# Scuttie/Few-Shot-Prompt-Learning-for-Vision-Language-Models-in-Imbalanced-Datasets

Hardware: AMD Instinct MI355X
Metric: CoCoOp ViT-B/16 16-shot train-step images/sec at 1/2/4/8 GPUs; eval images/sec (higher is better)
Workload: dtype fp32s

## Files before the change

### few-shot-prompt-learning-for-vision-language-models-in-imbalanced-datasets_amd/_native.py

```python
from __future__ import annotations

import ctypes
import hashlib
import os
import sys

_PKG = os.path.dirname(os.path.abspath(__file__))
LIB_PATH = os.environ.get("CLIPK_LIB") or os.path.join(_PKG, "libclipk.so")
_ROOT = os.path.dirname(_PKG)


def source_files():
    csrc = os.path.join(_PKG, "csrc")
    names = sorted(n for n in os.listdir(csrc) if n.endswith((".hip", ".h")) or n == "Makefile")
    rel = [("csrc/" + n, os.path.join(csrc, n)) for n in names]
    return rel + [("include/clipk.h", os.path.join(_ROOT, "include", "clipk.h"))]


def source_digest():
    h = hashlib.sha256()
    for rel, path in source_files():
        with open(path, "rb") as f:
            h.update(f"{hashlib.sha256(f.read()).hexdigest()}  {rel}\n".encode())
    return h.hexdigest()

F32, F16, BF16, F32S = 0, 1, 2, 3
PREFIX_CLS_GROUP0 = 1
PREFIX_SPLIT = 2
PREFIX_OUT_SPLIT = 4
ATTN_SPLIT = 1
ATTN_OUT_SPLIT = 2
F32S16 = 4
SPLIT_SCALE = 64.0
EPI_BIAS, EPI_BIAS_RES, EPI_BIAS_QGELU, EPI_DQGELU, EPI_NONE = 0, 1, 2, 3, 4
A_QGELU = 0x100
QGELU_DERIV = 0x200
OUT_SPLIT, A_SPLIT = 0x400, 0x800
ADAM_ADAM, ADAM_ADAMW, ADAM_AMSGRAD = 0, 1, 2
COLOR_BRIGHTNESS, COLOR_CONTRAST, COLOR_SATURATION, COLOR_HUE, COLOR_GRAYSCALE = 1, 2, 3, 4, 5
COLOR_MAX_OPS, COLOR_DESC = 5, 12
CONV_RES, CONV_RELU, CONV_OUT_F32 = 1, 2, 4
PROF_NONE, PROF_GEMM_FC, PROF_GEMM_ALL, PROF_ATTN, PROF_LN, PROF_GEMM_DGELU = 0, 1, 2, 3, 4, 5

_P = ctypes.c_void_p
_I = ctypes.c_int
_L = ctypes.c_long
_F = ctypes.c_float
_S = ctypes.c_size_t
_D = ctypes.c_double
_U = ctypes.c_uint

SIGNATURES = {
    "clipk_version": (ctypes.c_char_p, []),
    "clipk_source_digest": (ctypes.c_char_p, []),
    "clipk_strerror": (ctypes.c_char_p, [_I]),
    "clipk_device_arch_ok": (_I, []),
    "clipk_gemm": (_I, [_I, _I, _I, _I, _I, _I, _P, _I, _P, _I, _P, _P, _I, _P, _I, _P, _P, _I, _I, _P]),
    "clipk_gemm_auto_splits": (_I, [_I, _I, _I, _I]),
    "clipk_gemm_splitk_ws_bytes": (_S, [_I, _I, _I]),
    "clipk_gemm_splitk": (_I, [_I, _I, _I, _I, _I, _I, _P, _I, _P, _I, _P, _P, _I, _P, _I, _P, _I, _P, _S, _P]),
    "clipk_gemm_set_config": (_I, [_I]),
    "clipk_split_pack": (_I, [_I, _I, _P, _I, _P, _P]),
    "clipk_split_lo_zero": (_I, [_I, _I, _P, _P, _P]),
    "clipk_split_hi16": (_I, [_I, _I, _P, _P, _P]),
    "clipk_gemm_ln": (_I, [_I, _I, _I, _I, _I, _P, _I, _P, _I, _P, _P, _I, _P, _I, _P, _P, _P, _P, _P]),
    "clipk_ln_stats_merge": (_I, [_I, _I, _P, _P, _P, _P, _P]),
    "clipk_gemm_ln_merge_fused": (_I, [_I, _I, _I, _I]),
    "clipk_gemm_split_tile_rows": (_I, [_I, _I, _I, _I, _I]),
    "clipk_gemm_t256_cost": (_D, [_I, _I, _I]),
    "clipk_gemm_ln_stats_split": (_I, [_I, _I, _I, _I, _I, _P, _I, _P, _I, _P, _P, _I, _P, _I, _P, _P, _P, _P]),
    "clipk_gemm_ln_gamma": (_I, [_I, _I, _I, _I, _I, _P, _I, _P, _I, _P, _P, _I, _P, _P, _P, _P, _P]),
    "clipk_gemm_ln_merge": (_I, [_I, _I, _I, _I, _I, _P, _I, _P, _I, _P, _P, _I, _P, _P, _P, _P, _P, _P, _P]),
    "clipk_image_resample": (_I, [_I, _I, _I, _P, _P, _P, _P, _P, _P, _I, _P, _P]),
    "clipk_image_color": (_I, [_I, _I, _P, _P, _P, _P, _P, _I, _P, _P]),
    "clipk_gemm_stamps": (_I, [_P, _S]),
    "clipk_layernorm_fwd": (_I, [_I, _I, _I, _P, _I, _P, _P, _P, _P, _I, _P, _P, _P]),
    "clipk_layernorm_bwd": (_I, [_I, _I, _I, _P, _I, _P, _I, _P, _P, _P, _P, _P, _I, _P, _P, _I, _P, _I, _P]),
    "clipk_layernorm_fwd_x": (_I, [_I, _I, _I, _I, _P, _I, _P, _P, _P, _P, _I, _P, _P, _P]),
    "clipk_layernorm_bwd_x": (_I, [_I, _I, _I, _I, _P, _I, _P, _I, _P, _P, _P, _P, _P, _I, _P, _P, _I, _P, _I, _P]),
    "clipk_layernorm_bwd_x2": (_I, [_I, _I, _I, _I, _P, _I, _P, _I, _P, _P, _P, _P, _P, _I, _I, _P, _P, _I, _P, _I, _P]),
    "clipk_attention_fwd": (_I, [_I, _I, _I, _I, _I, _P, _I, _P, _I, _P, _P]),
    "clipk_attention_fwd_ex": (_I, [_I, _I, _I, _I, _I, _P, _I, _P, _I, _P, _I, _P]),
    "clipk_attention_bwd": (_I, [_I, _I, _I, _I, _I, _I, _P, _I, _P, _I, _P, _I, _P, _P, _I, _P]),
    "clipk_im2col": (_I, [_I, _I, _I, _I, _I, _P, _P, _P]),
    "clipk_vit_embed_ln": (_I, [_I, _I, _I, _P, _P, _P, _P, _P, _P, _P]),
    "clipk_prompt_assemble": (_I, [_I, _I, _I, _I, _P, _P, _P, _L, _L, _P, _P, _P, _P]),
    "clipk_ctx_grad": (_I, [_I, _I, _I, _I, _I, _I, _P, _P, _P, _P]),
    "clipk_prompt_assemble_rows": (_I, [_I, _I, _I, _I, _I, _P, _P, _P, _P, _L, _L, _P, _P, _P, _P]),
    "clipk_ctx_grad_rows": (_I, [_I, _I, _I, _I, _P, _P, _P, _P, _P]),
    "clipk_ctx_bias_grad_rows": (_I, [_I, _I, _I, _I, _P, _P, _P, _P, _P, _P]),
    "clipk_attention_prefix_fwd": (_I, [_I, _I, _I, _I, _I, _P, _P, _I, _P, _I, _P, _I, _P, _P]),
    "clipk_attention_prefix_ws_bytes": (_S, [_I, _I, _I]),
    "clipk_attention_prefix_bwd": (_I, [_I, _I, _I, _I, _I, _I, _P, _P, _I, _P, _I, _P, _I, _P, _I, _P, _P,
                                        _I, _P, _S, _P]),
    "clipk_attention_prefix_fwd_ex": (_I, [_I, _I, _I, _I, _I, _P, _P, _I, _P, _I, _P, _I, _P, _I, _P]),
    "clipk_attention_prefix_bwd_ex": (_I, [_I, _I, _I, _I, _I, _I, _P, _P, _I, _P, _I, _P, _I, _P, _I, _P, _P,
                                           _I, _P, _S, _I, _P]),
    "clipk_cosine_logits_fwd": (_I, [_I, _I, _I, _I, _F, _P, _P, _P, _P, _P, _P]),
    "clipk_cosine_logits_bwd": (_I, [_I, _I, _I, _I, _F, _P, _P, _P, _P, _P, _P, _P]),
    "clipk_ce_loss": (_I, [_I, _I, _P, _P, _P, _F, _I, _F, _P, _P, _P]),
    "clipk_ce_loss_reduce": (_I, [_I, _I, _P, _P, _P, _F, _I, _F, _I, _P, _P, _P, _P]),
    "clipk_ce_loss_mix": (_I, [_I, _I, _P, _P, _P, _F, _P, _F, _I, _F, _I, _P, _P, _P, _P]),
    "clipk_mixup_images": (_I, [_I, _L, _P, _P, _P, _P, _F, _F, _P, _P]),
    "clipk_ntxent_ws_bytes": (_S, [_I, _I]),
    "clipk_ntxent_loss": (_I, [_I, _I, _P, _P, _F, _F, _P, _P, _P, _P, _P]),
    "clipk_src_head_ws_bytes": (_S, [_I, _I, _I]),
    "clipk_src_head": (_I, [_I, _I, _I, _P, _P, _P, _P, _P, _P, _P, _F, _I, _F, _F, _F, _F, _F, _P, _P, _P, _P, _P,
                            _P]),
    "clipk_probe_head_ws_bytes": (_S, [_I, _I, _I]),
    "clipk_probe_head": (_I, [_I, _I, _I, _P, _P, _P, _P, _P, _F, _I, _I, _F, _F, _P, _P, _P, _P, _P, _P]),
    "clipk_meta_net_fwd": (_I, [_I, _I, _I, _I, _P, _P, _P, _P, _P, _P, _P, _P]),
    "clipk_meta_net_fwd_norm": (_I, [_I, _I, _I, _I, _P, _P, _P, _P, _P, _P, _P, _P, _P]),
    "clipk_status_take": (_I, [_P, _P, _P]),
    "clipk_meta_net_bwd": (_I, [_I, _I, _I, _I, _P, _P, _P, _P, _P, _P, _P, _P, _P, _P]),
    "clipk_sgd_step": (_I, [_L, _P, _P, _P, _F, _F, _F, _I, _P]),
    "clipk_sgd_step_multi": (_I, [_I, _P, _P, _P, _P, _P, _F, _F, _F, _P]),
    "clipk_sgd_step_multi_scaled": (_I, [_I, _P, _P, _P, _P, _P, _F, _F, _F, _F, _P]),
    "clipk_sgd_step_multi_if": (_I, [_I, _P, _P, _P, _P, _P, _F, _F, _F, _F, _P, _I, _P]),
    "clipk_adam_step_multi": (_I, [_I, _P, _P, _P, _P, _P, _P, _P, _P, _D, _D, _D, _D, _D, _I, _F, _P, _I, _P]),
    "clipk_cast": (_I, [_I, _L, _P, _P, _P]),
    "clipk_rows_copy": (_I, [_I, _I, _P, _P, _P, _P, _P]),
    "clipk_vit_embed_ln_vpt": (_I, [_I, _I, _I, _I, _P, _P, _P, _P, _P, _P, _P, _P]),
    "clipk_rows_inject": (_I, [_I, _I, _I, _I, _P, _P, _P, _I, _P]),
    "clipk_rows_collect": (_I, [_I, _I, _I, _I, _P, _I, _P, _I, _I, _P, _P, _I, _I, _P]),
    "clipk_encoder_set_deep_prompts": (_I, [_P, _I, _I, _I, _P, _P, _P]),
    "clipk_encoder_set_input_rows": (_I, [_P, _I]),
    "clipk_encoder_set_ln_fold": (_I, [_P, _P]),
    "clipk_encoder_set_split": (_I, [_P, _I]),
    "clipk_encoder_set_split_target": (_I, [_P, _I]),
    "clipk_encoder_set_status": (_I, [_P, _P]),
    "clipk_lora_merge": (_I, [_I, _I, _I, _I, _U, _F, _I, _I, _P, _P, _P, _P, _P, _P]),
    "clipk_lora_wgrad_ws_bytes": (_S, [_I, _I, _I]),
    "clipk_lora_wgrad": (_I, [_I, _I, _I, _I, _I, _I, _F, _P, _P, _P, _P, _P, _P, _P, _P, _P, _P, _P, _S, _P]),
    "clipk_encoder_set_lora": (_I, [_P, _I, _I, _U, _F, _P, _P, _P, _P]),
    "clipk_vit_prompted_saved_bytes": (_S, [_P, _I, _I]),
    "clipk_vit_prompted_ws_bytes": (_S, [_P, _I, _I]),
    "clipk_vit_forward_prompted": (_I, [_P, _I, _P, _I, _P, _P, _P, _S, _P, _S, _P]),
    "clipk_vit_backward_prompted": (_I, [_P, _I, _I, _P, _P, _P, _P, _S, _P, _P, _S, _P]),
    "clipk_encoder_create": (_I, [_I, _I, _I, _I, _I, _I, _P, _P, _P]),
    "clipk_encoder_destroy": (None, [_P]),
    "clipk_text_saved_bytes": (_S, [_P, _I, _I]),
    "clipk_text_ws_bytes": (_S, [_P, _I, _I]),
    "clipk_text_forward": (_I, [_P, _I, _I, _P, _P, _P, _P, _S, _P, _S, _P]),
    "clipk_text_bwd_ws_bytes": (_S, [_P, _I, _I]),
    "clipk_text_backward": (_I, [_P, _I, _I, _P, _P, _P, _S, _P, _P, _S, _P]),
    "clipk_text_packed_saved_bytes": (_S, [_P, _I, _I, _I]),
    "clipk_text_packed_ws_bytes": (_S, [_P, _I, _I, _I]),
    "clipk_text_packed_bwd_ws_bytes": (_S, [_P, _I, _I, _I, _I]),
    "clipk_text_forward_packed": (_I, [_P, _I, _I, _I, _I, _I, _P, _P, _P, _P, _P, _P, _S, _P, _S, _P]),
    "clipk_text_backward_packed": (_I, [_P, _I, _I, _I, _I, _I, _P, _P, _P, _P, _P, _S, _P, _P, _S, _P]),
    "clipk_vision_create": (_I, [_I, _I, _I, _I, _I, _I, _I, _P, _P, _P]),
    "clipk_vit_ws_bytes": (_S, [_P, _I]),
    "clipk_vit_forward": (_I, [_P, _I, _P, _P, _P, _S, _P]),
    "clipk_conv2d_nhwc": (_I, [_I, _I, _I, _I, _I, _I, _I, _I, _P, _P, _P, _P, _P, _P, _P]),
    "clipk_im2col_3x3s2": (_I, [_I, _I, _I, _P, _P, _P]),
    "clipk_avgpool2_nhwc": (_I, [_I, _I, _I, _I, _I, _P, _P, _P]),
    "clipk_attnpool_ws_bytes": (_S, [_I, _I, _I, _I]),
    "clipk_attnpool": (_I, [_I, _I, _I, _I, _I, _I, _P, _P, _P, _P, _P, _P, _P, _P, _P, _P, _S, _P]),
    "clipk_resnet_create": (_I, [_I, _P, _I, _I, _I, _P, _I, _P]),
    "clipk_resnet_destroy": (None, [_P]),
    "clipk_resnet_ws_bytes": (_S, [_P, _I]),
    "clipk_resnet_forward": (_I, [_P, _I, _P, _P, _P, _S, _P]),
    "clipk_prof_enable": (_I, [_I]),
    "clipk_prof_read": (_I, [_P, _P, _P]),
    "clipk_prof_sites_enable": (_I, [_I]),
    "clipk_prof_sites_read": (_I, [_I, _P, _P, _P, _P, _P, _P]),
}

PROF_NAME_LEN = 32


def prof_sites_read(max_sites: int = 64):
    lib = load()
    names = ctypes.create_string_buffer(max_sites * PROF_NAME_LEN)
    ms = (ctypes.c_double * max_sites)()
    cnt = (ctypes.c_long * max_sites)()
    fl = (ctypes.c_double * max_sites)()
    by = (ctypes.c_double * max_sites)()
    n = ctypes.c_int()
    check(lib.clipk_prof_sites_read(max_sites, names, ms, cnt, fl, by, ctypes.byref(n)), "clipk_prof_sites_read")
    out = {}
    for i in range(n.value):
        nm = names.raw[i * PROF_NAME_LEN:(i + 1) * PROF_NAME_LEN].split(b"\0", 1)[0].decode()
        if cnt[i]:
            out[nm] = (ms[i], cnt[i], fl[i], by[i])
    return out

_lib = None


class ClipkError(RuntimeError):
    pass


def load():
    global _lib
    if _lib is not None:
        return _lib
    if not os.path.isfile(LIB_PATH):
        raise ClipkError(f"{LIB_PATH} is missing: the HIP extension is not built "
                         f"(run `python __graft_entry__.py` or `make -C csrc`). No CPU fallback exists.")
    lib = ctypes.CDLL(LIB_PATH)
    for name, (res, args) in SIGNATURES.items():
        fn = getattr(lib, name)
        fn.restype = res
        fn.argtypes = args
    built = lib.clipk_source_digest().decode()
    tree = source_digest()
    if built != tree:
        raise ClipkError(f"{LIB_PATH} was built from other sources than this tree (library digest {built[:16]}, "
                         f"tree {tree[:16]}): rebuild it (`python __graft_entry__.py` or `make -C csrc`)")
    _lib = lib
    return lib


def library_digest():
    return load().clipk_source_digest().decode()


def strerror(rc: int) -> str:
    return load().clipk_strerror(rc).decode()


def check(rc: int, what: str):
    if rc != 0:
        raise ClipkError(f"{what} failed: {strerror(rc)} (status {rc})")


def call(name: str, *args):
    rc = getattr(load(), name)(*args)
    check(rc, name)
    return rc


if __name__ == "__main__" and sys.argv[1:] == ["--digest-header"]:
    print(f'#define CLIPK_SOURCE_DIGEST "{source_digest()}"')
```

### few-shot-prompt-learning-for-vision-language-models-in-imbalanced-datasets_amd/csrc/attention_prefix.hip

```cpp
#include <cstdlib>

#include "attn_common.h"

namespace clipk {

constexpr int kValuChunkMin = 4;

static int chunk_env(const char* name, int def) {
  const char* e = getenv(name);
  const int v = e ? atoi(e) : def;
  return v >= 1 && v <= 16 ? v : def;
}
static int lds_slots();
static int fwd_chunk() { static int c = chunk_env("CLIPK_PREFIX_FWD_CHUNK", lds_slots() ? 4 : 8); return c; }
static int bwd_chunk() { static int c = chunk_env("CLIPK_PREFIX_BWD_CHUNK", 16); return c; }
static int prefix_num_cus() {
  static int n = 0;
  if (!n) {
    int dev = 0, v = 0;
    n = (hipGetDevice(&dev) == hipSuccess &&
         hipDeviceGetAttribute(&v, hipDeviceAttributeMultiprocessorCount, dev) == hipSuccess && v > 0)
            ? v
            : 256;
  }
// ... 698 lines not shown
__device__ __forceinline__ void f32_stage_prefix(const float* __restrict__ qkv, size_t row0, int P, int ldq, int col,
                                                 int W, float* sKp, float* sVp) {
  for (int i = threadIdx.x; i < P * 16; i += WPB * 64) {
    const int j = i >> 4, c = i & 15;
    const float* b = qkv + (row0 + j) * ldq + col + 4 * c;
    reinterpret_cast<f32x4*>(sKp)[i] = *reinterpret_cast<const f32x4*>(b + W);
    reinterpret_cast<f32x4*>(sVp)[i] = *reinterpret_cast<const f32x4*>(b + 2 * W);
  }
}
static size_t f32_prefix_lds(int P) { return (size_t)2 * P * 64 * sizeof(float); }

template <int WPB>
__global__ __launch_bounds__(WPB * 64) void attn_prefix_fwd_f32(
    int G, int P, int R, int ntiles, const int* __restrict__ tiles, const int* __restrict__ row_first, int H,
    int nchunk, int uc, const float* __restrict__ qkv, int ldq, float* __restrict__ out, int ldo,
    float* __restrict__ lse, int cls0) {
  extern __shared__ CLIPK_LDS_ALIGN float sPre[];
  float* const sKp = sPre;
  float* const sVp = sPre + P * 64;
  __shared__ CLIPK_LDS_ALIGN float sK[WPB][16 * 64], sV[WPB][16 * 64];
  int g, h, k, w;
  f32_block<WPB>(H, nchunk, g, h, k, w);
  const int W = H * 64;
  f32_stage_prefix<WPB>(qkv, (size_t)g * R, P, ldq, h * 64, W, sKp, sVp);
  __syncthreads();
  if (k >= nchunk) return;
  const int lane = threadIdx.x & 63, r = lane >> 2, s = lane & 3;
  float* sk = sK[w];
  float* sv = sV[w];
  const int u_end = min((k + 1) * uc, ntiles + 1);
  float qn[16], kn[16], vn[16];
  int t0n, nn, pren, rrn, firstn;
  auto fetch = [&](int u) {
    f32_unit(tiles, row_first, P, u, r, t0n, nn, pren, rrn, firstn);
    const float* qp = qkv + ((cls0 && u > 0 ? 0 : (size_t)g * R) + t0n + rrn) * ldq + h * 64 + kSl * s;
    ld16x(qp, qn);
    ld16x(qp + W, kn);
    ld16x(qp + 2 * W, vn);
  };
  if (k * uc < u_end) fetch(k * uc);
  for (int u = k * uc; u < u_end; ++u) {
    const int t0 = t0n, n = nn, pre = pren, rr = rrn, first = firstn;
    const size_t row = (size_t)g * R + t0 + rr;
    float q[16];
#pragma unroll
    for (int d = 0; d < 16; ++d) q[d] = qn[d] * kScale;
    st16x(sk + r * 64 + kSl * s, kn);
    st16x(sv + r * 64 + kSl * s, vn);
    lds_sync();
    if (u + 1 < u_end) fetch(u + 1);
    float sp[16], so[16], m = -INFINITY;
#pragma unroll
    for (int j = 0; j < 16; ++j) {
      if (j < pre) {
        float kv[16];
        ld16x(sKp + j * 64 + kSl * s, kv);
        sp[j] = quad_sum(dot16(q, kv));
        m = fmaxf(m, sp[j]);
      }
    }
#pragma unroll
    for (int j = 0; j < 16; ++j) {
      if (j < n) {
        float kv[16];
        ld16x(sk + j * 64 + kSl * s, kv);
        const float sc = quad_sum(dot16(q, kv));
        so[j] = (j <= rr && j >= first) ? sc : -INFINITY;
        m = fmaxf(m, so[j]);
      }
    }
    float l = 0.f, o[16];
#pragma unroll
    for (int d = 0; d < 16; ++d) o[d] = 0.f;
#pragma unroll
    for (int j = 0; j < 16; ++j) {
      if (j < pre) {
        float vv[16];
        ld16x(sVp + j * 64 + kSl * s, vv);
        const float p = __expf(sp[j] - m);
        l += p;
#pragma unroll
        for (int d = 0; d < 16; ++d) o[d] = fmaf(p, vv[d], o[d]);
      }
    }
#pragma unroll
    for (int j = 0; j < 16; ++j) {
      if (j < n) {
        float vv[16];
        ld16x(sv + j * 64 + kSl * s, vv);
        const float p = __expf(so[j] - m);
        l += p;
#pragma unroll
        for (int d = 0; d < 16; ++d) o[d] = fmaf(p, vv[d], o[d]);
      }
    }
    if (r < n) {
      const float inv = 1.0f / l;
#pragma unroll
      for (int d = 0; d < 16; ++d) o[d] *= inv;
      st16x(out + row * ldo + h * 64 + kSl * s, o);
      if (lse && s == 0) lse[row * H + h] = m + __logf(l);
    }
    lds_sync();
  }
}

template <int WPB, bool OS = false>
__global__ __launch_bounds__(WPB * 64, 2) void attn_prefix_bwd_f32(
    int G, int P, int R, int ntiles, const int* __restrict__ tiles, const int* __restrict__ row_first, int H,
    int nchunk, int uc, const float* __restrict__ qkv, int ldq, const float* __restrict__ o_fwd, int ldof,
    const float* __restrict__ dout, int lddo, const float* __restrict__ lse, float* __restrict__ dqkv, int lddq,
    float* __restrict__ part, int cls0) {
  extern __shared__ CLIPK_LDS_ALIGN float sPre[];
  float* const sKp = sPre;
  float* const sVp = sPre + P * 64;
  constexpr int RS = 68, PS = 33;
  __shared__ CLIPK_LDS_ALIGN float sA[WPB][16 * RS], sB[WPB][16 * RS];
  __shared__ CLIPK_LDS_ALIGN float sP[WPB][16 * PS], sS[WPB][16 * PS];
  int g, h, k, w;
  f32_block<WPB>(H, nchunk, g, h, k, w);
  const int W = H * 64;
  f32_stage_prefix<WPB>(qkv, (size_t)g * R, P, ldq, h * 64, W, sKp, sVp);
  __syncthreads();
  if (k >= nchunk) return;
  const int lane = threadIdx.x & 63, r = lane >> 2, s = lane & 3;
  float* sa = sA[w];
  float* sb = sB[w];
  float* sp = sP[w];
  float* ss = sS[w];
  float akp[16], avp[16];
#pragma unroll
  for (int d = 0; d < 16; ++d) { akp[d] = 0.f; avp[d] = 0.f; }
  const int u_end = min((k + 1) * uc, ntiles + 1);
  float qn[16], dOn[16], on[16], kn[16], vn[16], lin = 0.f;
  int t0n, nn, pren, rrn, firstn;
  auto fetch = [&](int u) {
    f32_unit(tiles, row_first, P, u, r, t0n, nn, pren, rrn, firstn);
    const size_t rw = (size_t)g * R + t0n + rrn;
    const float* qp = qkv + ((cls0 && u > 0 ? 0 : (size_t)g * R) + t0n + rrn) * ldq + h * 64 + kSl * s;
    ld16x(qp, qn);
    ld16x(dout + rw * lddo + h * 64 + kSl * s, dOn);
    ld16x(o_fwd + rw * ldof + h * 64 + kSl * s, on);
    ld16x(qp + W, kn);
    ld16x(qp + 2 * W, vn);
    lin = lse[rw * H + h];
  };
  if (k * uc < u_end) fetch(k * uc);
  for (int u = k * uc; u < u_end; ++u) {
    const int t0 = t0n, n = nn, pre = pren, rr = rrn, first = firstn;
    const bool qok = r < n;
    const size_t row = (size_t)g * R + t0 + rr;
    float q[16], dO[16];
#pragma unroll
    for (int d = 0; d < 16; ++d) {
      q[d] = qn[d] * kScale;
      dO[d] = dOn[d];
    }
    const float Di = quad_sum(dot16(dO, on));
    const float li = lin;
    st16x(sa + r * RS + kSl * s, kn);
    st16x(sb + r * RS + kSl * s, vn);
    lds_sync();
    if (u + 1 < u_end) fetch(u + 1);
    float dq[16];
#pragma unroll
    for (int d = 0; d < 16; ++d) dq[d] = 0.f;
    auto key = [&](const float* kr, const float* vr, bool ok, int col) {
      float kv[16], vv[16];
      ld16x(kr + kSl * s, kv);
      ld16x(vr + kSl * s, vv);
      const float sc = quad_sum(dot16(q, kv));
      const float dp = quad_sum(dot16(dO, vv));
      const float p = ok ? __expf(sc - li) : 0.f;
      const float ds = p * (dp - Di);
#pragma unroll
      for (int d = 0; d < 16; ++d) dq[d] = fmaf(ds, kv[d], dq[d]);
      if (s == 0) {
        sp[r * PS + col] = p;
        ss[r * PS + col] = ds;
      }
    };
    for (int j = 0; j < pre; ++j) key(sKp + j * 64, sVp + j * 64, qok, j);
    for (int j = 0; j < n; ++j) key(sa + j * RS, sb + j * RS, qok && j <= rr && j >= first, 16 + j);
    if (qok) {
#pragma unroll
      for (int d = 0; d < 16; ++d) dq[d] *= kScale;
      if constexpr (OS) st16x_split(dqkv + row * lddq + h * 64 + kSl * s, dq, s);
      else st16x(dqkv + row * lddq + h * 64 + kSl * s, dq);
    }
    st16x(sa + r * RS + kSl * s, q);
    st16x(sb + r * RS + kSl * s, dO);
    lds_sync();
    auto keysum = [&](int col, float* dk, float* dv) {
      for (int i = 0; i < n; ++i) {
        const float pv = sp[i * PS + col], dsv = ss[i * PS + col];
        float a[16], b[16];
        ld16x(sa + i * RS + kSl * s, a);
        ld16x(sb + i * RS + kSl * s, b);
#pragma unroll
        for (int d = 0; d < 16; ++d) {
          dk[d] = fmaf(dsv, a[d], dk[d]);
          dv[d] = fmaf(pv, b[d], dv[d]);
        }
      }
    };
    if (u == 0) {
      keysum(16 + r, akp, avp);
    } else {
      float dk[16], dv[16];
#pragma unroll
      for (int d = 0; d < 16; ++d) { dk[d] = 0.f; dv[d] = 0.f; }
      for (int i = 0; i < n; ++i) {
        const float pv = sp[i * PS + 16 + r], dsv = ss[i * PS + 16 + r];
        const float pp = sp[i * PS + r], dsp = ss[i * PS + r];
        float a[16], b[16];
        ld16x(sa + i * RS + kSl * s, a);
        ld16x(sb + i * RS + kSl * s, b);
#pragma unroll
        for (int d = 0; d < 16; ++d) {
          dk[d] = fmaf(dsv, a[d], dk[d]);
          dv[d] = fmaf(pv, b[d], dv[d]);
          akp[d] = fmaf(dsp, a[d], akp[d]);
          avp[d] = fmaf(pp, b[d], avp[d]);
        }
      }
      if (qok) {
        if constexpr (OS) {
          st16x_split(dqkv + row * lddq + W + h * 64 + kSl * s, dk, s);
          st16x_split(dqkv + row * lddq + 2 * W + h * 64 + kSl * s, dv, s);
        } else {
          st16x(dqkv + row * lddq + W + h * 64 + kSl * s, dk);
          st16x(dqkv + row * lddq + 2 * W + h * 64 + kSl * s, dv);
        }
      }
    }
    lds_sync();
  }
  if (r < P) {
    float* pb = part + (((size_t)g * nchunk + k) * 16 + r) * (2 * W) + h * 64 + kSl * s;
    st16x(pb, akp);
    st16x(pb + W, avp);
  }
}


struct Parts8 { s16x8 hi[2], lo[2]; };

__device__ __forceinline__ void ld_frag32(const float* p, f32x4 (&x)[4]) {
#pragma unroll
  for (int i = 0; i < 4; ++i) x[i] = *reinterpret_cast<const f32x4*>(p + 16 * i);
}
__device__ __forceinline__ void split_frag(const f32x4 (&x)[4], Parts8& o) {
#pragma unroll
  for (int kk = 0; kk < 2; ++kk) {
    f16x8 h, l;
#pragma unroll
    for (int j = 0; j < 2; ++j)
#pragma unroll
      for (int e = 0; e < 4; ++e) {
        const float v = x[2 * kk + j][e];
        const f16 hh = (f16)v;
        h[4 * j + e] = hh;
        l[4 * j + e] = (f16)(v - (float)hh);
      }
    o.hi[kk] = __builtin_bit_cast(s16x8, h);
    o.lo[kk] = __builtin_bit_cast(s16x8, l);
  }
}
__device__ __forceinline__ void st_parts(const Parts8& f, short* thi, short* tlo, int r16, int g4) {
#pragma unroll
  for (int i = 0; i < 4; ++i) {
    const int o = r16 * TRS + 16 * i + 4 * g4;
    const s16x8 h = f.hi[i >> 1], l = f.lo[i >> 1];
    const int b = 4 * (i & 1);
    *reinterpret_cast<s16x4*>(thi + o) = (s16x4){h[b], h[b + 1], h[b + 2], h[b + 3]};
    *reinterpret_cast<s16x4*>(tlo + o) = (s16x4){l[b], l[b + 1], l[b + 2], l[b + 3]};
  }
}
__device__ __forceinline__ f32x4 mfma32_s3(const Parts8& a, const Parts8& b, f32x4 c) {
#pragma unroll
  for (int kk = 0; kk < 2; ++kk) {
    c = mfma32_t<f16>(a.lo[kk], b.hi[kk], c);
    c = mfma32_t<f16>(a.hi[kk], b.lo[kk], c);
  }
#pragma unroll
  for (int kk = 0; kk < 2; ++kk) c = mfma32_t<f16>(a.hi[kk], b.hi[kk], c);
  return c;
}
__device__ __forceinline__ f32x4 mfma16_s3(s16x4 ah, s16x4 al, s16x4 bh, s16x4 bl, f32x4 c) {
  c = mfma16_t<f16>(al, bh, c);
  c = mfma16_t<f16>(ah, bl, c);
  return mfma16_t<f16>(ah, bh, c);
}
__device__ __forceinline__ void ld_prefix_parts(const float* p, bool ok, Parts8& o) {
  f32x4 x[4];
  ld_frag32(p, x);
#pragma unroll
  for (int i = 0; i < 4; ++i)
    if (!ok) x[i] = (f32x4){0.f, 0.f, 0.f, 0.f};
  split_frag(x, o);
}
constexpr int kSplitFwdWpc = 12, kSplitBwdWpc = 8;

template <int WPB, bool OS>
__global__ __launch_bounds__(WPB * 64) void attn_prefix_fwd_split(
    int G, int P, int R, int ntiles, const int* __restrict__ tiles, const int* __restrict__ row_first, int H,
    int nchunk, int uc, const float* __restrict__ qkv, int ldq, float* __restrict__ out, int ldo,
    float* __restrict__ lse, int cls0) {
  __shared__ CLIPK_LDS_ALIGN short sm[WPB][4][16 * TRS];
  const int lane = threadIdx.x & 63, w = threadIdx.x >> 6;
  const int r16 = lane & 15, g4 = lane >> 4;
  const int wid = blockIdx.x * WPB + w;
  if (wid >= G * nchunk * H) return;
  const int h = wid % H, k = (wid / H) % nchunk, g = wid / (H * nchunk);
  const int W = H * 64;
  short* sVpH = sm[w][0];
  short* sVpL = sm[w][1];
  short* sVoH = sm[w][2];
  short* sVoL = sm[w][3];
  const size_t gR = (size_t)g * R;
  const float* qh = qkv + h * 64 + 4 * g4;
  const int u_begin = k * uc, u_end = min((k + 1) * uc, ntiles + 1);
  const int tab = load_tile_table(tiles, ntiles, u_begin, lane);

  f32x4 qn[4], kn[4], vn[4];
  int firstn = 0;
  auto fetch = [&](int u) {
    int t0, n, pre;
    tile_info(tab, P, u, u_begin, t0, n, pre);
    const int rl = t0 + min(r16, n - 1);
    const float* qp = qh + ((cls0 && u > 0 ? 0 : gR) + rl) * ldq;
    ld_frag32(qp, qn);
    ld_frag32(qp + W, kn);
    ld_frag32(qp + 2 * W, vn);
    firstn = u == 0 ? 0 : row_first[rl] - t0;
  };
  if (u_begin < u_end) fetch(u_begin);
  Parts8 kp;
  {
    const bool pok = r16 < P;
    const float* pp = qh + (gR + (pok ? r16 : 0)) * ldq;
    Parts8 vp;
    ld_prefix_parts(pp + W, pok, kp);
    ld_prefix_parts(pp + 2 * W, pok, vp);
    st_parts(vp, sVpH, sVpL, r16, g4);
  }
  for (int u = u_begin; u < u_end; ++u) {
    int t0, n, pre;
    tile_info(tab, P, u, u_begin, t0, n, pre);
    const int first = firstn;
    const bool qok = r16 < n;
    Parts8 q, ko;
    {
      Parts8 vo;
      split_frag(qn, q);
      split_frag(kn, ko);
      split_frag(vn, vo);
      lds_fence();
      st_parts(vo, sVoH, sVoL, r16, g4);
    }
    const f32x4 z = {0.f, 0.f, 0.f, 0.f};
    const f32x4 sp = mfma32_s3(kp, q, z);
    const f32x4 so = mfma32_s3(ko, q, z);
    __builtin_amdgcn_sched_barrier(0);
    if (u + 1 < u_end) fetch(u + 1);
    float vp[4], vq[4], mx = -INFINITY;
#pragma unroll
    for (int r = 0; r < 4; ++r) {
      const int key = 4 * g4 + r;
      vp[r] = key < pre ? sp[r] * kScale : -INFINITY;
      vq[r] = (key <= r16 && key >= first) ? so[r] * kScale : -INFINITY;
      mx = fmaxf(mx, fmaxf(vp[r], vq[r]));
    }
    mx = xmax4(mx);
    float ep[4], eo[4], ps = 0.f;
#pragma unroll
    for (int r = 0; r < 4; ++r) {
      ep[r] = __expf(vp[r] - mx);
      eo[r] = __expf(vq[r] - mx);
      ps += ep[r] + eo[r];
    }
    ps = xsum4(ps);
    s16x4 bpH, bpL, boH, boL;
    split_pack4(ep[0] * kPScale, ep[1] * kPScale, ep[2] * kPScale, ep[3] * kPScale, bpH, bpL);
    split_pack4(eo[0] * kPScale, eo[1] * kPScale, eo[2] * kPScale, eo[3] * kPScale, boH, boL);
    const float inv = kPInv / ps;
    lds_fence();
    float* orow = out + (gR + t0 + r16) * ldo + h * 64;
#pragma unroll
    for (int t = 0; t < 4; ++t) {
      f32x4 o = mfma16_s3(tr_read(sVpH, 4 * g4, 16 * t, lane), tr_read(sVpL, 4 * g4, 16 * t, lane), bpH, bpL, z);
      o = mfma16_s3(tr_read(sVoH, 4 * g4, 16 * t, lane), tr_read(sVoL, 4 * g4, 16 * t, lane), boH, boL, o);
      store_acc16<OS>(orow, o * inv, t, qok, g4);
    }
    if (lse && g4 == 0 && qok) lse[(gR + t0 + r16) * H + h] = mx + __logf(ps);
  }
}

template <int WPB, bool OS>
__global__ __launch_bounds__(WPB * 64, 2) void attn_prefix_bwd_split(
    int G, int P, int R, int ntiles, const int* __restrict__ tiles, const int* __restrict__ row_first, int H,
    int nchunk, int uc, const float* __restrict__ qkv, int ldq, const float* __restrict__ dout, int lddo,
    const float* __restrict__ lse, float* __restrict__ dqkv, int lddq, float* __restrict__ part, int cls0) {
  __shared__ CLIPK_LDS_ALIGN short sm[WPB][8][16 * TRS];
  const int lane = threadIdx.x & 63, w = threadIdx.x >> 6;
  const int r16 = lane & 15, g4 = lane >> 4;
  const int wid = blockIdx.x * WPB + w;
  if (wid >= G * nchunk * H) return;
  const int h = wid % H, k = (wid / H) % nchunk, g = wid / (H * nchunk);
  const int W = H * 64;
  short* tKpH = sm[w][0];
  short* tKpL = sm[w][1];
  short* tKoH = sm[w][2];
  short* tKoL = sm[w][3];
  short* tQH = sm[w][4];
  short* tQL = sm[w][5];
  short* tDH = sm[w][6];
  short* tDL = sm[w][7];
  const size_t gR = (size_t)g * R;
  const float* qh = qkv + h * 64 + 4 * g4;
  const float* dh = dout + h * 64 + 4 * g4;
  const float* lse_h = lse + h;
  const int u_begin = k * uc, u_end = min((k + 1) * uc, ntiles + 1);
  const int tab = load_tile_table(tiles, ntiles, u_begin, lane);

  f32x4 qn[4], kn[4], vn[4], dn[4];
  float l2n = 0.f;
  int first2n = 0;
  auto fetch = [&](int u) {
    int t0, n, pre;
    tile_info(tab, P, u, u_begin, t0, n, pre);
    const int rl = t0 + min(r16, n - 1);
    const float* qp = qh + ((cls0 && u > 0 ? 0 : gR) + rl) * ldq;
    ld_frag32(qp, qn);
    ld_frag32(qp + W, kn);
    ld_frag32(qp + 2 * W, vn);
    ld_frag32(dh + (gR + rl) * lddo, dn);
    l2n = lse_h[(gR + rl) * H];
    first2n = u == 0 ? 0 : row_first[rl] - t0;
  };
  if (u_begin < u_end) fetch(u_begin);
  Parts8 kp, vp;
  {
    const bool pok = r16 < P;
    const float* pp = qh + (gR + (pok ? r16 : 0)) * ldq;
    ld_prefix_parts(pp + W, pok, kp);
    ld_prefix_parts(pp + 2 * W, pok, vp);
    st_parts(kp, tKpH, tKpL, r16, g4);
  }
  const f32x4 z = {0.f, 0.f, 0.f, 0.f};
  f32x4 dkp[4], dvp[4];
#pragma unroll
  for (int t = 0; t < 4; ++t) {
    dkp[t] = z;
    dvp[t] = z;
  }
  for (int u = u_begin; u < u_end; ++u) {
    int t0, n, pre;
    tile_info(tab, P, u, u_begin, t0, n, pre);
    const bool own_is_prefix = u == 0;
    const bool qok = r16 < n;
    const float l2 = l2n;
    const int first2 = first2n;
    f32x4 s1p, s2p, p1p, p2p, s1o, s2o, p1o, p2o;
    {
      Parts8 q, ko, vo, d;
      split_frag(qn, q);
      split_frag(kn, ko);
      split_frag(vn, vo);
      split_frag(dn, d);
      lds_fence();
      st_parts(q, tQH, tQL, r16, g4);
      st_parts(ko, tKoH, tKoL, r16, g4);
      st_parts(d, tDH, tDL, r16, g4);
      s1p = mfma32_s3(q, kp, z);
      s2p = mfma32_s3(kp, q, z);
      p1p = mfma32_s3(d, vp, z);
      p2p = mfma32_s3(vp, d, z);
      s1o = mfma32_s3(q, ko, z);
      s2o = mfma32_s3(ko, q, z);
      p1o = mfma32_s3(d, vo, z);
      p2o = mfma32_s3(vo, d, z);
    }
    __builtin_amdgcn_sched_barrier(0);
    if (u + 1 < u_end) fetch(u + 1);
    float P2p[4], P2o[4], Dsum = 0.f;
#pragma unroll
    for (int r = 0; r < 4; ++r) {
      const int j = 4 * g4 + r;
      P2p[r] = (qok && j < pre) ? __expf(s2p[r] * kScale - l2) : 0.f;
      P2o[r] = (qok && j <= r16 && j >= first2) ? __expf(s2o[r] * kScale - l2) : 0.f;
      Dsum += P2p[r] * p2p[r] + P2o[r] * p2o[r];
    }
    Dsum = xsum4(Dsum);
    s16x4 bTpH, bTpL, bToH, bToL;
    split_pack4(P2p[0] * (p2p[0] - Dsum), P2p[1] * (p2p[1] - Dsum), P2p[2] * (p2p[2] - Dsum),
                P2p[3] * (p2p[3] - Dsum), bTpH, bTpL);
    split_pack4(P2o[0] * (p2o[0] - Dsum), P2o[1] * (p2o[1] - Dsum), P2o[2] * (p2o[2] - Dsum),
                P2o[3] * (p2o[3] - Dsum), bToH, bToL);
    float P1p[4], P1o[4], dS1p[4], dS1o[4];
#pragma unroll
    for (int r = 0; r < 4; ++r) {
      const int i = 4 * g4 + r;
      const bool iok = i < n;
      const float Di = __shfl(Dsum, i, 64), l1 = __shfl(l2, i, 64);
      const int first1 = __shfl(first2, i, 64);
      P1p[r] = (iok && r16 < pre) ? __expf(s1p[r] * kScale - l1) : 0.f;
      P1o[r] = (iok && r16 <= i && r16 >= first1) ? __expf(s1o[r] * kScale - l1) : 0.f;
      dS1p[r] = P1p[r] * (p1p[r] - Di);
      dS1o[r] = P1o[r] * (p1o[r] - Di);
    }
    s16x4 bPpH, bPpL, bPoH, bPoL, bSpH, bSpL, bSoH, bSoL;
    split_pack4(P1p[0] * kPScale, P1p[1] * kPScale, P1p[2] * kPScale, P1p[3] * kPScale, bPpH, bPpL);
    split_pack4(P1o[0] * kPScale, P1o[1] * kPScale, P1o[2] * kPScale, P1o[3] * kPScale, bPoH, bPoL);
    split_pack4(dS1p[0], dS1p[1], dS1p[2], dS1p[3], bSpH, bSpL);
    split_pack4(dS1o[0], dS1o[1], dS1o[2], dS1o[3], bSoH, bSoL);
    lds_fence();
    float* orow = dqkv + (gR + t0 + r16) * lddq + h * 64;
    f32x4 acc[4];
#pragma unroll
    for (int t = 0; t < 4; ++t) {
      acc[t] = mfma16_s3(tr_read(tKpH, 4 * g4, 16 * t, lane), tr_read(tKpL, 4 * g4, 16 * t, lane), bTpH, bTpL, z);
      acc[t] = mfma16_s3(tr_read(tKoH, 4 * g4, 16 * t, lane), tr_read(tKoL, 4 * g4, 16 * t, lane), bToH, bToL, acc[t]);
    }
    store_acc64<OS>(orow, acc, kScale, qok, g4);
#pragma unroll
    for (int t = 0; t < 4; ++t) {
      const s16x4 aH = tr_read(tQH, 4 * g4, 16 * t, lane), aL = tr_read(tQL, 4 * g4, 16 * t, lane);
      dkp[t] = mfma16_s3(aH, aL, bSpH, bSpL, dkp[t]);
      acc[t] = mfma16_s3(aH, aL, bSoH, bSoL, z);
      if (own_is_prefix) dkp[t] += acc[t];
    }
    if (!own_is_prefix) store_acc64<OS>(orow + W, acc, kScale, qok, g4);
#pragma unroll
    for (int t = 0; t < 4; ++t) {
      const s16x4 aH = tr_read(tDH, 4 * g4, 16 * t, lane), aL = tr_read(tDL, 4 * g4, 16 * t, lane);
      dvp[t] = mfma16_s3(aH, aL, bPpH, bPpL, dvp[t]);
      acc[t] = mfma16_s3(aH, aL, bPoH, bPoL, z);
      if (own_is_prefix) dvp[t] += acc[t];
    }
    if (!own_is_prefix) store_acc64<OS>(orow + 2 * W, acc, kPInv, qok, g4);
  }
  float* pb = part + ((size_t)g * nchunk + k) * 16 * (2 * W);
  if (r16 < P) {
#pragma unroll
    for (int t = 0; t < 4; ++t) {
      float* dst = pb + (size_t)r16 * 2 * W + h * 64 + 16 * t + 4 * g4;
      *reinterpret_cast<f32x4*>(dst) = dkp[t] * kScale;
      *reinterpret_cast<f32x4*>(dst + W) = dvp[t] * kPInv;
    }
  }
}

template <typename TG>
__global__ __launch_bounds__(256) void prefix_kv_reduce(int P, int R, int W, int nchunk,
                                                        const float* __restrict__ part,
                                                        TG* __restrict__ dqkv, int lddq) {
  const int g = blockIdx.x / P, p = blockIdx.x % P;
  const int col = blockIdx.y * 256 + threadIdx.x;
  if (col >= 2 * W) return;
  const float* src = part + ((size_t)g * nchunk * 16 + p) * 2 * W + col;
  const size_t cs = (size_t)16 * 2 * W;
  float a0 = 0.f, a1 = 0.f, a2 = 0.f, a3 = 0.f;
  int k = 0;
  for (; k + 16 <= nchunk; k += 16) {
    float v[16];
#pragma unroll
    for (int i = 0; i < 16; ++i) v[i] = src[(k + i) * cs];
#pragma unroll
    for (int i = 0; i < 16; i += 4) {
      a0 += v[i];
      a1 += v[i + 1];
      a2 += v[i + 2];
      a3 += v[i + 3];
    }
  }
  for (; k + 4 <= nchunk; k += 4) {
    a0 += src[k * cs];
    a1 += src[(k + 1) * cs];
    a2 += src[(k + 2) * cs];
    a3 += src[(k + 3) * cs];
  }
  for (; k < nchunk; ++k) a0 += src[k * cs];
  const float acc = (a0 + a1) + (a2 + a3);
  dqkv[((size_t)g * R + p) * lddq + W + col] = (TG)acc;
}

__global__ __launch_bounds__(256) void prefix_kv_reduce_split(int P, int R, int W, int nchunk,
                                                              const float* __restrict__ part,
                                                              float* __restrict__ dqkv, int lddq) {
  const int g = blockIdx.x / P, p = blockIdx.x % P;
  const int col = blockIdx.y * 256 + threadIdx.x;
  if (col >= 2 * W) return;
  const float* src = part + ((size_t)g * nchunk * 16 + p) * 2 * W + col;
  const size_t cs = (size_t)16 * 2 * W;
  float a0 = 0.f, a1 = 0.f, a2 = 0.f, a3 = 0.f;
  int k = 0;
  for (; k + 16 <= nchunk; k += 16) {
    float v[16];
#pragma unroll
    for (int i = 0; i < 16; ++i) v[i] = src[(k + i) * cs];
#pragma unroll
    for (int i = 0; i < 16; i += 4) {
      a0 += v[i];
      a1 += v[i + 1];
      a2 += v[i + 2];
      a3 += v[i + 3];
    }
  }
  for (; k + 4 <= nchunk; k += 4) {
    a0 += src[k * cs];
    a1 += src[(k + 1) * cs];
    a2 += src[(k + 2) * cs];
    a3 += src[(k + 3) * cs];
  }
  for (; k < nchunk; ++k) a0 += src[k * cs];
  _Float16 hi, lo;
  split_parts((a0 + a1) + (a2 + a3), hi, lo);
  const int c = W + col;
  _Float16* grp = reinterpret_cast<_Float16*>(dqkv + ((size_t)g * R + p) * lddq + (c & ~7));
  grp[c & 7] = hi;
  grp[8 + (c & 7)] = lo;
}

template <typename T>
static int prefix_fwd(int G, int P, int R, int ntiles, const int* tiles, const int* row_first, int H,
                      const void* qkv, int ldq, void* out, int ldo, float* lse, hipStream_t st, int cls0) {
  if constexpr (sizeof(T) == 2) {
    const int uc = fwd_chunk();
    const int nchunk = n_chunks(ntiles, uc);
    const long waves = (long)G * nchunk * H;
    if (const int ns = lds_slots()) {
      const int wpb = lds_wpb();
      auto go = [&](auto kern) {
        hipLaunchKernelGGL(kern, dim3((waves + wpb - 1) / wpb), dim3(64 * wpb), 0, st, G, P, R, ntiles, tiles,
                           row_first, H, nchunk, uc, (const T*)qkv, ldq, (T*)out, ldo, lse, cls0);
      };
#define CLIPK_LDS_GO(K, T_, ...)                                                               \
  if (ns == 2) { if (wpb == 1) go(K<T_, 2, 1 __VA_ARGS__>); else if (wpb == 2) go(K<T_, 2, 2 __VA_ARGS__>); \
                 else go(K<T_, 2, 4 __VA_ARGS__>); }                                                 \
  else { if (wpb == 1) go(K<T_, 3, 1 __VA_ARGS__>); else if (wpb == 2) go(K<T_, 3, 2 __VA_ARGS__>);     \
         else go(K<T_, 3, 4 __VA_ARGS__>); }
      CLIPK_LDS_GO(attn_prefix_fwd_lds, T)
      CLIPK_CHECK_LAUNCH();
      return CLIPK_OK;
    }
    const int b = fwd_batch();
    const int wpb = prefix_wpb();
    auto go = [&](auto kern) {
      hipLaunchKernelGGL(kern, dim3((waves + wpb - 1) / wpb), dim3(64 * wpb), 0, st, G, P, R, ntiles, tiles,
                         row_first, H, nchunk, uc, (const T*)qkv, ldq, (T*)out, ldo, lse, cls0);
    };
    if (wpb == 8) {
      if (b == 1) go(attn_prefix_fwd_mfma<T, 1, 8>);
      else if (b == 2) go(attn_prefix_fwd_mfma<T, 2, 8>);
      else go(attn_prefix_fwd_mfma<T, 4, 8>);
    } else {
      if (b == 1) go(attn_prefix_fwd_mfma<T, 1>);
      else if (b == 2) go(attn_prefix_fwd_mfma<T, 2>);
      else go(attn_prefix_fwd_mfma<T, 4>);
    }
  } else {
    const int uc = f32_uc(G, ntiles, H, kF32FwdWpc);
    const int nchunk = n_chunks(ntiles, uc);
    auto go = [&](auto kern, int wpb) {
      const long blocks = (long)G * ((nchunk + wpb - 1) / wpb) * H;
      hipLaunchKernelGGL(kern, dim3(blocks), dim3(64 * wpb), f32_prefix_lds(P), st, G, P, R, ntiles, tiles, row_first,
                         H, nchunk, uc, (const float*)qkv, ldq, (float*)out, ldo, lse, cls0);
    };
    const int wpb = f32_wpb();
    if (wpb == 2) go(attn_prefix_fwd_f32<2>, 2);
    else if (wpb == 8) go(attn_prefix_fwd_f32<8>, 8);
    else go(attn_prefix_fwd_f32<4>, 4);
  }
  CLIPK_CHECK_LAUNCH();
  return CLIPK_OK;
}

template <typename T, typename TG, bool OS = false>
static int prefix_bwd(int G, int P, int R, int ntiles, const int* tiles, const int* row_first, int H,
                      const void* qkv, int ldq, const void* ofwd, int ldof, const void* dout, int lddo,
                      const float* lse, void* dqkv, int lddq, float* part, hipStream_t st, int cls0) {
  static_assert(!OS || (sizeof(T) == 4 && sizeof(TG) == 4), "pre-split dQ|dK|dV: the fp32 backward");
  constexpr bool mfma = sizeof(TG) == 2 && sizeof(T) == 2;
  const int uc = mfma ? bwd_uc(G, ntiles, H) : f32_uc(G, ntiles, H, kF32BwdWpc);
  const int nchunk = n_chunks(ntiles, uc);
  const long waves = (long)G * nchunk * H;
  if constexpr (mfma && __is_same(T, TG)) {
    if (const int ns = lds_slots()) {
      const int wpb = lds_wpb();
      auto go = [&](auto kern) {
        hipLaunchKernelGGL(kern, dim3((waves + wpb - 1) / wpb), dim3(64 * wpb), 0, st, G, P, R, ntiles, tiles,
                           row_first, H, nchunk, uc, (const T*)qkv, ldq, (const T*)dout, lddo, lse, (T*)dqkv,
                           lddq, part, cls0);
      };
      CLIPK_LDS_GO(attn_prefix_bwd_lds, T)
      CLIPK_CHECK_LAUNCH();
      const int W = H * 64;
      hipLaunchKernelGGL((prefix_kv_reduce<TG>), dim3(G * P, (2 * W + 255) / 256), dim3(256), 0, st, P, R, W,
                         nchunk, part, (TG*)dqkv, lddq);
      CLIPK_CHECK_LAUNCH();
      return CLIPK_OK;
    }
  }
  if constexpr (mfma) {
    const int wpb = prefix_wpb();
    auto go = [&](auto kern) {
      hipLaunchKernelGGL(kern, dim3((waves + wpb - 1) / wpb), dim3(64 * wpb), 0, st, G, P, R, ntiles, tiles,
                         row_first, H, nchunk, uc, (const T*)qkv, ldq, (const TG*)dout, lddo, lse, (TG*)dqkv,
                         lddq, part, cls0);
    };
    if (wpb == 8) {
      if (bwd_batch() == 1) go(attn_prefix_bwd_mfma<T, TG, 1, 8>);
      else go(attn_prefix_bwd_mfma<T, TG, 2, 8>);
    } else {
      if (bwd_batch() == 1) go(attn_prefix_bwd_mfma<T, TG, 1>);
      else go(attn_prefix_bwd_mfma<T, TG, 2>);
    }
  } else {
    static_assert(mfma || (sizeof(T) == 4 && sizeof(TG) == 4), "fp32 backward");
    auto go = [&](auto kern, int wpb) {
      const long blocks = (long)G * ((nchunk + wpb - 1) / wpb) * H;
      hipLaunchKernelGGL(kern, dim3(blocks), dim3(64 * wpb), f32_prefix_lds(P), st, G, P, R, ntiles, tiles, row_first,
                         H, nchunk, uc, (const float*)qkv, ldq, (const float*)ofwd, ldof, (const float*)dout, lddo,
                         lse, (float*)dqkv, lddq, part, cls0);
    };
    const int wpb = f32_wpb();
    if (wpb == 2) go(attn_prefix_bwd_f32<2, OS>, 2);
    else if (wpb == 8) go(attn_prefix_bwd_f32<8, OS>, 8);
    else go(attn_prefix_bwd_f32<4, OS>, 4);
  }
  CLIPK_CHECK_LAUNCH();
  const int W = H * 64;
  if constexpr (OS)
    hipLaunchKernelGGL(prefix_kv_reduce_split, dim3(G * P, (2 * W + 255) / 256), dim3(256), 0, st, P, R, W,
                       nchunk, part, (float*)dqkv, lddq);
  else
    hipLaunchKernelGGL((prefix_kv_reduce<TG>), dim3(G * P, (2 * W + 255) / 256), dim3(256), 0, st, P, R, W,
                       nchunk, part, (TG*)dqkv, lddq);
  CLIPK_CHECK_LAUNCH();
  return CLIPK_OK;
}

static int prefix_fwd_split(int G, int P, int R, int ntiles, const int* tiles, const int* row_first, int H,
                            const void* qkv, int ldq, void* out, int ldo, float* lse, hipStream_t st, int cls0,
                            bool out_split) {
  constexpr int WPB = 4;
  const int uc = f32_uc(G, ntiles, H, kSplitFwdWpc);
  const int nchunk = n_chunks(ntiles, uc);
  const long waves = (long)G * nchunk * H;
  if (out_split)
    hipLaunchKernelGGL((attn_prefix_fwd_split<WPB, true>), dim3((waves + WPB - 1) / WPB), dim3(64 * WPB), 0, st, G, P, R,
                       ntiles, tiles, row_first, H, nchunk, uc, (const float*)qkv, ldq, (float*)out, ldo, lse, cls0);
  else
    hipLaunchKernelGGL((attn_prefix_fwd_split<WPB, false>), dim3((waves + WPB - 1) / WPB), dim3(64 * WPB), 0, st, G, P, R,
                       ntiles, tiles, row_first, H, nchunk, uc, (const float*)qkv, ldq, (float*)out, ldo, lse, cls0);
  CLIPK_CHECK_LAUNCH();
  return CLIPK_OK;
}

template <bool OS>
static int prefix_bwd_split(int G, int P, int R, int ntiles, const int* tiles, const int* row_first, int H,
                            const void* qkv, int ldq, const void* dout, int lddo, const float* lse, void* dqkv,
                            int lddq, float* part, hipStream_t st, int cls0) {
  static_assert(kSplitBwdWpc == kF32BwdWpc, "workspace sized by the fp32 backward's chunking");
  constexpr int WPB = 2;
  const int uc = f32_uc(G, ntiles, H, kSplitBwdWpc);
  const int nchunk = n_chunks(ntiles, uc);
  const long waves = (long)G * nchunk * H;
  hipLaunchKernelGGL((attn_prefix_bwd_split<WPB, OS>), dim3((waves + WPB - 1) / WPB), dim3(64 * WPB), 0, st, G, P, R,
                     ntiles, tiles, row_first, H, nchunk, uc, (const float*)qkv, ldq, (const float*)dout, lddo, lse,
                     (float*)dqkv, lddq, part, cls0);
  CLIPK_CHECK_LAUNCH();
  const int W = H * 64;
  if constexpr (OS)
    hipLaunchKernelGGL(prefix_kv_reduce_split, dim3(G * P, (2 * W + 255) / 256), dim3(256), 0, st, P, R, W,
                       nchunk, part, (float*)dqkv, lddq);
  else
    hipLaunchKernelGGL((prefix_kv_reduce<float>), dim3(G * P, (2 * W + 255) / 256), dim3(256), 0, st, P, R, W,
                       nchunk, part, (float*)dqkv, lddq);
  CLIPK_CHECK_LAUNCH();
  return CLIPK_OK;
}

}

using namespace clipk;

static int prefix_shape_ok(int G, int P, int R, int ntiles, int heads, int ldq) {
  return G > 0 && P >= 1 && P <= 16 && ntiles >= 1 && R > P && heads > 0 &&
         (long)G * R * (long)(ldq > 3 * heads * 64 ? ldq : 3 * heads * 64) < (1L << 31);
}

extern "C" size_t clipk_attention_prefix_ws_bytes(int G, int ntiles, int heads) {
  if (G <= 0 || ntiles <= 0 || heads <= 0) return 0;
  const int ub = bwd_uc(G, ntiles, heads), uf = f32_uc(G, ntiles, heads, kF32BwdWpc);
  const int uc = ub < uf ? ub : uf;
  return (size_t)G * n_chunks(ntiles, uc) * 16 * 2 * heads * 64 * sizeof(float);
}

constexpr int kPrefixFlags = CLIPK_PREFIX_CLS_GROUP0 | CLIPK_PREFIX_SPLIT;
constexpr int kPrefixFwdFlags = kPrefixFlags | CLIPK_PREFIX_OUT_SPLIT;
static int prefix_fwd_call(int dtype, int G, int P, int R, int ntiles, const int* tiles, const int* row_first,
                           int heads, const void* qkv, int ldqkv, void* out, int ldo, float* lse, int flags,
                           void* stream) {
  if (!tiles || !row_first || !qkv || !out) return CLIPK_EINVAL;
  if (flags & ~kPrefixFwdFlags) return CLIPK_EINVAL;
  if ((flags & CLIPK_PREFIX_SPLIT) && dtype != CLIPK_F32) return CLIPK_EINVAL;
  if ((flags & CLIPK_PREFIX_OUT_SPLIT) && (!(flags & CLIPK_PREFIX_SPLIT) || ldo % 8)) return CLIPK_EINVAL;
  if (!prefix_shape_ok(G, P, R, ntiles, heads, ldqkv) || ldqkv < 3 * heads * 64 || ldo < heads * 64 ||
      ldqkv % 8 || ldo % 8)
    return CLIPK_ESHAPE;
  hipStream_t st = (hipStream_t)stream;
  const int c0 = (flags & CLIPK_PREFIX_CLS_GROUP0) ? 1 : 0;
  if (flags & CLIPK_PREFIX_SPLIT)
    return prefix_fwd_split(G, P, R, ntiles, tiles, row_first, heads, qkv, ldqkv, out, ldo, lse, st, c0,
                            (flags & CLIPK_PREFIX_OUT_SPLIT) != 0);
  switch (dtype) {
    case CLIPK_F16: return prefix_fwd<f16>(G, P, R, ntiles, tiles, row_first, heads, qkv, ldqkv, out, ldo, lse, st, c0);
    case CLIPK_BF16: return prefix_fwd<bf16>(G, P, R, ntiles, tiles, row_first, heads, qkv, ldqkv, out, ldo, lse, st, c0);
    case CLIPK_F32: return prefix_fwd<float>(G, P, R, ntiles, tiles, row_first, heads, qkv, ldqkv, out, ldo, lse, st, c0);
    default: return CLIPK_EDTYPE;
  }
}

extern "C" int clipk_attention_prefix_fwd(int dtype, int G, int P, int R, int ntiles, const int* tiles,
                                          const int* row_first, int heads, const void* qkv, int ldqkv,
                                          void* out, int ldo, float* lse, void* stream) {
  return prefix_fwd_call(dtype, G, P, R, ntiles, tiles, row_first, heads, qkv, ldqkv, out, ldo, lse, 0, stream);
}

extern "C" int clipk_attention_prefix_fwd_ex(int dtype, int G, int P, int R, int ntiles, const int* tiles,
                                             const int* row_first, int heads, const void* qkv, int ldqkv,
                                             void* out, int ldo, float* lse, int flags, void* stream) {
  return prefix_fwd_call(dtype, G, P, R, ntiles, tiles, row_first, heads, qkv, ldqkv, out, ldo, lse, flags, stream);
}

static int prefix_bwd_call(int dtype, int grad_dtype, int G, int P, int R, int ntiles, const int* tiles,
                           const int* row_first, int heads, const void* qkv, int ldqkv, const void* ofwd, int ldof,
                           const void* dout, int lddo, const float* lse, void* dqkv, int lddqkv, void* ws,
                           size_t ws_bytes, int flags, void* stream) {
  if (!tiles || !row_first || !qkv || !ofwd || !dout || !lse || !dqkv || !ws) return CLIPK_EINVAL;
  if (flags & ~kPrefixFlags) return CLIPK_EINVAL;
  if ((flags & CLIPK_PREFIX_SPLIT) && (dtype != CLIPK_F32 || (grad_dtype != CLIPK_F32 && grad_dtype != CLIPK_F32S)))
    return CLIPK_EINVAL;
  if (!prefix_shape_ok(G, P, R, ntiles, heads, lddqkv) || ldqkv < 3 * heads * 64 || lddqkv < 3 * heads * 64 ||
      ldof < heads * 64 || lddo < heads * 64)
    return CLIPK_ESHAPE;
  if (ws_bytes < clipk_attention_prefix_ws_bytes(G, ntiles, heads)) return CLIPK_EWORKSPACE;
  hipStream_t st = (hipStream_t)stream;
  float* part = (float*)ws;
  const int c0 = (flags & CLIPK_PREFIX_CLS_GROUP0) ? 1 : 0;
  if (flags & CLIPK_PREFIX_SPLIT) {
    if (ldqkv % 4 || lddo % 4 || lddqkv % 4) return CLIPK_ESHAPE;
    if (grad_dtype == CLIPK_F32S) {
      if (lddqkv % 8) return CLIPK_ESHAPE;
      return prefix_bwd_split<true>(G, P, R, ntiles, tiles, row_first, heads, qkv, ldqkv, dout, lddo, lse, dqkv,
                                    lddqkv, part, st, c0);
    }
    return prefix_bwd_split<false>(G, P, R, ntiles, tiles, row_first, heads, qkv, ldqkv, dout, lddo, lse, dqkv,
                                   lddqkv, part, st, c0);
  }
#define CLIPK_PBWD(TT, TGG)                                                                           \
  return prefix_bwd<TT, TGG>(G, P, R, ntiles, tiles, row_first, heads, qkv, ldqkv, ofwd, ldof, dout, lddo, \
                             lse, dqkv, lddqkv, part, st, c0)
  if (dtype == CLIPK_F16 && grad_dtype == CLIPK_BF16) CLIPK_PBWD(f16, bf16);
  if (dtype == CLIPK_F16 && grad_dtype == CLIPK_F16) CLIPK_PBWD(f16, f16);
  if (dtype == CLIPK_BF16 && grad_dtype == CLIPK_BF16) CLIPK_PBWD(bf16, bf16);
  if (dtype == CLIPK_F32 && grad_dtype == CLIPK_F32) CLIPK_PBWD(float, float);
  if (dtype == CLIPK_F32 && grad_dtype == CLIPK_F32S) {
    if (lddqkv % 8) return CLIPK_ESHAPE;
    return prefix_bwd<float, float, true>(G, P, R, ntiles, tiles, row_first, heads, qkv, ldqkv, ofwd, ldof, dout,
                                          lddo, lse, dqkv, lddqkv, part, st, c0);
  }
#undef CLIPK_PBWD
  return CLIPK_EDTYPE;
}

extern "C" int clipk_attention_prefix_bwd(int dtype, int grad_dtype, int G, int P, int R, int ntiles,
                                          const int* tiles, const int* row_first, int heads,
                                          const void* qkv, int ldqkv, const void* ofwd, int ldof,
                                          const void* dout, int lddo, const float* lse, void* dqkv,
                                          int lddqkv, void* ws, size_t ws_bytes, void* stream) {
  return prefix_bwd_call(dtype, grad_dtype, G, P, R, ntiles, tiles, row_first, heads, qkv, ldqkv, ofwd, ldof, dout,
                         lddo, lse, dqkv, lddqkv, ws, ws_bytes, 0, stream);
}

extern "C" int clipk_attention_prefix_bwd_ex(int dtype, int grad_dtype, int G, int P, int R, int ntiles,
                                             const int* tiles, const int* row_first, int heads,
                                             const void* qkv, int ldqkv, const void* ofwd, int ldof,
                                             const void* dout, int lddo, const float* lse, void* dqkv,
                                             int lddqkv, void* ws, size_t ws_bytes, int flags, void* stream) {
  return prefix_bwd_call(dtype, grad_dtype, G, P, R, ntiles, tiles, row_first, heads, qkv, ldqkv, ofwd, ldof, dout,
                         lddo, lse, dqkv, lddqkv, ws, ws_bytes, flags, stream);
}
```

### few-shot-prompt-learning-for-vision-language-models-in-imbalanced-datasets_amd/csrc/encoder.hip

```cpp
#include <vector>
#include <array>
#include <cstring>
#include <new>
#include <cstdlib>
#include <algorithm>

#include "common.h"

struct DeepPrompts {
  int n_deep = 0, n_ctx = 0, n_per = 0;
  const int* rows = nullptr;
  const float* prompts = nullptr;
  float* grads = nullptr;
};

struct clipk_encoder {
  int kind;
  int W, layers, heads, E, act, grad;
  int res, patch, Kp, Limg;
  std::vector<std::array<const void*, 16>> lw;
  std::array<const void*, 8> head;
  DeepPrompts deep;
  int prefix_input = 0;
  std::vector<std::array<const void*, 6>> fold;
  int split = 0;
  int split_target = 7;
  int* status = nullptr;
  struct Lora {
    int rank = 0, proj_mask = 0;
    unsigned layer_mask = 0;
    float scale = 0.f;
    const float *A = nullptr, *B = nullptr;
    float *dA = nullptr, *dB = nullptr;
  } lora;
  mutable int o_saved_split = 0;
};

namespace clipk {

static inline size_t esize(int dt) { return (dt == CLIPK_F32 || dt == CLIPK_F32S || dt == CLIPK_F32S16) ? 4 : 2; }

static thread_local int t_split = 0;
static thread_local bool t_osplit = false;
struct SplitScope {
  int prev;
  bool prev_o;
  explicit SplitScope(const clipk_encoder* e) : prev(t_split), prev_o(t_osplit) { t_split = e->split; t_osplit = false; }
  ~SplitScope() { t_split = prev; t_osplit = prev_o; }
};
static inline size_t align_up(size_t x) { return (x + 255) & ~size_t(255); }

static int res_dtype(const clipk_encoder* e) {
  static const bool force32 = getenv("CLIPK_TEXT_RES32") != nullptr;
  return (e->act == CLIPK_F32 || force32) ? CLIPK_F32 : e->act;
}

struct Carver {
  char* base;
  size_t off = 0;
  explicit Carver(void* b) : base((char*)b) {}
  void* take(size_t bytes) {
    void* p = base ? base + off : nullptr;
    off += align_up(bytes);
    return p;
  }
};

struct ProfState {
  int kind = CLIPK_PROF_NONE;
  bool sites = false;
  std::vector<std::pair<hipEvent_t, hipEvent_t>> ev;
  std::vector<double> work, bytes;
  std::vector<int> site;
  std::vector<const char*> names;
  size_t used = 0;
};
static ProfState g_prof;

static int site_index(const char* name) {
  for (size_t i = 0; i < g_prof.names.size(); ++i)
    if (std::strcmp(g_prof.names[i], name) == 0) return (int)i;
  g_prof.names.push_back(name);
  return (int)g_prof.names.size() - 1;
}

struct ProfScope {
  bool on = false;
  hipStream_t st;
  size_t idx = 0;
  ProfScope(int cls, hipStream_t s, double work, const char* site = nullptr, double bytes = 0.0) : st(s) {
    bool take = false;
    if (g_prof.sites) {
      take = site != nullptr;
    } else if (g_prof.kind != CLIPK_PROF_NONE && cls != CLIPK_PROF_NONE) {
      const bool is_gemm = cls == CLIPK_PROF_GEMM_FC || cls == CLIPK_PROF_GEMM_ALL || cls == CLIPK_PROF_GEMM_DGELU;
      take = g_prof.kind == cls || (g_prof.kind == CLIPK_PROF_GEMM_ALL && is_gemm);
    }
    if (!take) return;
    if (g_prof.used == g_prof.ev.size()) {
      hipEvent_t a, b;
      if (hipEventCreate(&a) != hipSuccess || hipEventCreate(&b) != hipSuccess) return;
      g_prof.ev.push_back({a, b});
      g_prof.work.push_back(0.0);
      g_prof.bytes.push_back(0.0);
      g_prof.site.push_back(-1);
    }
    idx = g_prof.used++;
    g_prof.work[idx] = work;
    g_prof.bytes[idx] = bytes;
    g_prof.site[idx] = site ? site_index(site) : -1;
    on = hipEventRecord(g_prof.ev[idx].first, st) == hipSuccess;
  }
  ~ProfScope() {
    if (on) (void)hipEventRecord(g_prof.ev[idx].second, st);
  }
};

#define TRY(x)                 \
  do {                         \
    int _rc = (x);             \
    if (_rc != CLIPK_OK) return _rc; \
  } while (0)

static double gemm_bytes(int in, int out, int epi, int M, int N, int K, bool has_o2, int auxdt) {
  const double a = esize(in), o = esize(out), wb = in == CLIPK_F32S16 ? 2.0 : a;
  double b = (double)M * K * a + (double)N * K * wb + (double)M * N * o * (has_o2 ? 2 : 1);
  const int e = epi & ~(CLIPK_A_QGELU | CLIPK_QGELU_DERIV | CLIPK_A_SPLIT | CLIPK_OUT_SPLIT | CLIPK_OUT2_SPLIT_GAMMA);
  if (e == CLIPK_EPI_BIAS_RES) b += (double)M * N * o;
  if (e == CLIPK_EPI_DQGELU) b += (double)M * N * esize(auxdt);
  return b;
}

static int gemm(int in, int out, int epi, int M, int N, int K, const void* A, const void* B,
                const float* bias, const void* res, void* o, void* o2, const void* aux, int auxdt,
                hipStream_t st, int prof_cls, void* sk = nullptr, size_t skb = 0, const char* site = nullptr) {
  if (t_split && in == CLIPK_F32) in = t_split == 2 ? CLIPK_F32S16 : CLIPK_F32S;
  ProfScope ps(prof_cls, st, 2.0 * M * N * K, site,
               site ? gemm_bytes(in, out, epi, M, N, K, o2 != nullptr, auxdt) : 0.0);
  if (sk && (epi & ~CLIPK_QGELU_DERIV) != CLIPK_EPI_DQGELU)
    return clipk_gemm_splitk(in, out, epi, M, N, K, A, K, B, K, bias, res, N, o, N, o2, 0, sk, skb, st);
  return clipk_gemm(in, out, epi, M, N, K, A, K, B, K, bias, res, N, o, N, o2, aux, auxdt, N, st);
}

static size_t vit_splitk_bytes(int act, int rows, int D) {
  const int shapes[4][2] = {{3 * D, D}, {D, D}, {4 * D, D}, {D, 4 * D}};
  size_t best = 0;
  for (const auto& nk : shapes) {
    const size_t b = clipk_gemm_splitk_ws_bytes(rows, nk[0], clipk_gemm_auto_splits(act, rows, nk[0], nk[1]));
    best = b > best ? b : best;
  }
  return best;
}

struct TextBufs {
  std::vector<void*> X, Xm;
  std::vector<float*> mean1, rstd1, mean2, rstd2, lse;
  std::vector<void*> qkv, o, h;
  void* Xf = nullptr;
  float *meanf = nullptr, *rstdf = nullptr;
  void *xn = nullptr, *g = nullptr, *lnf = nullptr, *oc = nullptr, *xc = nullptr;
  float *lnst = nullptr, *tm = nullptr, *tr = nullptr, *rnb = nullptr;
  size_t saved_bytes = 0, ws_bytes = 0;
};

static TextBufs text_layout(const clipk_encoder* e, size_t rows, int nout, void* saved, void* ws, bool save,
                            int rd = -1) {
  TextBufs t;
  const size_t W = e->W, H = e->heads, a = esize(e->act), xs = esize(rd < 0 ? res_dtype(e) : rd);
  const int nl = e->layers;
  Carver sv(saved), wk(ws);
  Carver& S = save ? sv : wk;
  t.X.resize(nl + 1); t.Xm.resize(nl); t.mean1.resize(nl); t.rstd1.resize(nl);
  t.mean2.resize(nl); t.rstd2.resize(nl); t.lse.resize(nl); t.qkv.resize(nl); t.o.resize(nl);
  t.h.resize(nl);
  if (save) {
    for (int l = 0; l <= nl; ++l) t.X[l] = S.take(rows * W * xs);
    for (int l = 0; l < nl; ++l) {
      t.Xm[l] = S.take(rows * W * xs);
      t.mean1[l] = (float*)S.take(rows * 4); t.rstd1[l] = (float*)S.take(rows * 4);
      t.mean2[l] = (float*)S.take(rows * 4); t.rstd2[l] = (float*)S.take(rows * 4);
      t.lse[l] = (float*)S.take(rows * H * 4);
      t.qkv[l] = S.take(rows * 3 * W * a);
      t.o[l] = S.take(rows * W * a);
      t.h[l] = S.take(rows * 4 * W * a);
    }
    t.meanf = (float*)S.take((size_t)nout * 4);
    t.rstdf = (float*)S.take((size_t)nout * 4);
  } else {
    void* x0 = wk.take(rows * W * xs);
    void* x1 = wk.take(rows * W * xs);
    void* xm = wk.take(rows * W * xs);
    void* q = wk.take(rows * 3 * W * a);
    void* o = wk.take(rows * W * a);
    for (int l = 0; l <= nl; ++l) t.X[l] = (l & 1) ? x1 : x0;
    for (int l = 0; l < nl; ++l) {
      t.Xm[l] = xm; t.qkv[l] = q; t.o[l] = o; t.h[l] = nullptr;
      t.mean1[l] = t.rstd1[l] = t.mean2[l] = t.rstd2[l] = nullptr; t.lse[l] = nullptr;
    }
  }
  t.Xf = t.X[nl];
  t.xn = wk.take(rows * W * a);
  t.g = wk.take(rows * 4 * W * a);
  t.lnf = wk.take((size_t)nout * W * a);
  t.oc = wk.take((size_t)nout * W * a);
  t.xc = wk.take((size_t)nout * W * xs);
  t.lnst = (float*)wk.take(rows * (W / 64) * 8);
  t.tm = (float*)wk.take(rows * 4);
  t.tr = (float*)wk.take(rows * 4);
  t.rnb = (float*)wk.take(rows * 8);
  t.saved_bytes = save ? sv.off : 0;
  t.ws_bytes = wk.off;
  return t;
}

constexpr int kAmaxBlocks = 256;

struct TextBwdBufs {
  void *dtg, *dX_lp, *dh, *do_, *dqkv, *dxn;
  float* dlnf;
  float* gscale;
  void* part;
  void* lora;
  size_t lora_bytes;
  size_t bytes;
};

static TextBwdBufs text_bwd_layout(const clipk_encoder* e, size_t rows, int nout, size_t part_bytes,
                                   void* ws) {
  TextBwdBufs b;
  const size_t W = e->W, g = esize(e->grad);
  Carver c(ws);
  b.dtg = c.take((size_t)nout * e->E * g);
  b.dlnf = (float*)c.take((size_t)nout * W * 4);
  b.dX_lp = c.take(rows * W * g);
  b.dh = c.take(rows * 4 * W * g);
  b.dxn = c.take(rows * W * g);
  b.do_ = c.take(rows * W * g);
  b.dqkv = c.take(rows * 3 * W * g);
  b.part = part_bytes ? c.take(part_bytes) : nullptr;
  b.gscale = (float*)c.take((2 + kAmaxBlocks) * sizeof(float));
  b.lora_bytes = e->lora.rank > 0 ? clipk_lora_wgrad_ws_bytes((int)rows, (int)W, e->lora.rank) : 0;
  b.lora = b.lora_bytes ? c.take(b.lora_bytes) : nullptr;
  b.bytes = c.off;
  return b;
}

__global__ __launch_bounds__(256) void amax_partial_kernel(long n, const float* __restrict__ x,
                                                           float* __restrict__ part) {
  __shared__ float sm[4];
  float m = 0.f;
  for (long i = (long)blockIdx.x * 256 + threadIdx.x; i < n; i += (long)gridDim.x * 256) m = fmaxf(m, fabsf(x[i]));
  m = wave_max(m);
  if ((threadIdx.x & 63) == 0) sm[threadIdx.x >> 6] = m;
  __syncthreads();
  if (threadIdx.x == 0) part[blockIdx.x] = fmaxf(fmaxf(sm[0], sm[1]), fmaxf(sm[2], sm[3]));
}
__global__ __launch_bounds__(64) void grad_scale_pick_kernel(int nparts, int target, float* __restrict__ sc) {
  float m = 0.f;
  for (int i = threadIdx.x; i < nparts; i += 64) m = fmaxf(m, sc[2 + i]);
  m = wave_max(m);
  if (threadIdx.x == 0) {
    int ex = 0;
    if (m > 0.f && m < INFINITY) (void)frexpf(m, &ex);
    const int k = min(max(target - ex, -120), 120);
    sc[0] = ldexpf(1.0f, k);
    sc[1] = ldexpf(1.0f, -k);
  }
}
__global__ __launch_bounds__(256) void scale_by_kernel(long n, const float* __restrict__ x, float* __restrict__ y,
                                                       const float* __restrict__ sc, int which) {
  const float s = sc[which];
  for (long i = (long)blockIdx.x * 256 + threadIdx.x; i < n; i += (long)gridDim.x * 256) y[i] = x[i] * s;
}
static int grad_scale_in(const clipk_encoder* e, long n, const float* x, float* y, float* sc, hipStream_t st) {
  hipLaunchKernelGGL(amax_partial_kernel, dim3(kAmaxBlocks), dim3(256), 0, st, n, x, sc + 2);
  hipLaunchKernelGGL(grad_scale_pick_kernel, dim3(1), dim3(64), 0, st, kAmaxBlocks, e->split_target, sc);
  hipLaunchKernelGGL(scale_by_kernel, dim3((unsigned)std::min<long>((n + 255) / 256, 4096)), dim3(256), 0, st, n, x, y,
                     (const float*)sc, 0);
  CLIPK_CHECK_LAUNCH();
  return CLIPK_OK;
}
static int grad_scale_out(long n, float* x, const float* sc, hipStream_t st) {
  hipLaunchKernelGGL(scale_by_kernel, dim3((unsigned)std::min<long>((n + 255) / 256, 8192)), dim3(256), 0, st, n, x, x,
                     sc, 1);
  CLIPK_CHECK_LAUNCH();
  return CLIPK_OK;
}

__global__ __launch_bounds__(256) void finite_check_kernel(int nseg, long seg_len, long seg_stride,
                                                           const float* __restrict__ x, int* __restrict__ status,
                                                           int bit) {
  const long n = (long)nseg * seg_len;
  bool bad = false;
  for (long i = (long)blockIdx.x * 256 + threadIdx.x; i < n; i += (long)gridDim.x * 256)
    bad |= !__builtin_isfinite(x[(i / seg_len) * seg_stride + i % seg_len]);
  if (__any(bad) && (threadIdx.x & 63) == 0) atomicOr(status, bit);
}
static int split_check(const clipk_encoder* e, int nseg, long seg_len, long seg_stride, const float* x, int bit,
                       hipStream_t st) {
  if (!e->split || !e->status || nseg <= 0 || seg_len <= 0) return CLIPK_OK;
  const long nb = ((long)nseg * seg_len + 255) / 256;
  hipLaunchKernelGGL(finite_check_kernel, dim3((unsigned)std::min<long>(nb, 2048)), dim3(256), 0, st, nseg, seg_len,
                     seg_stride, x, e->status, bit);
  CLIPK_CHECK_LAUNCH();
  return CLIPK_OK;
}

struct SeqShape {
  int rows = 0, nout = 0;
  int nseq = 0, L = 0, causal = 0;
  bool packed = false;
  int G = 0, C = 0, P = 0, R = 0, ntiles = 0;
  const int* tiles = nullptr;
  const int* row_first = nullptr;
  static SeqShape plain(int nseq, int L, int causal) {
    SeqShape s;
    s.rows = nseq * L; s.nout = nseq; s.nseq = nseq; s.L = L; s.causal = causal;
    return s;
  }
  static SeqShape prefix(int G, int C, int P, int R, int ntiles, const int* tiles, const int* row_first) {
    SeqShape s;
    s.rows = G * R; s.nout = G * C; s.packed = true; s.causal = 1;
    s.G = G; s.C = C; s.P = P; s.R = R; s.ntiles = ntiles; s.tiles = tiles; s.row_first = row_first;
    return s;
  }
  size_t part_bytes(int heads) const { return packed ? clipk_attention_prefix_ws_bytes(G, ntiles, heads) : 0; }
};

constexpr int kPrefixSplitFwd = 1, kPrefixSplitBwd = 2, kPrefixSplitDefault = kPrefixSplitFwd | kPrefixSplitBwd;
static int prefix_split_flag(const clipk_encoder* e, int dir) {
  const char* s = getenv("CLIPK_PREFIX_SPLIT_ATTN");
  const int on = s ? atoi(s) : kPrefixSplitDefault;
  return (on & dir) && e->split != 0 && e->act == CLIPK_F32 ? CLIPK_PREFIX_SPLIT : 0;
}
static bool prefix_split_bwd(const clipk_encoder* e, const SeqShape& sh, int gd) {
  return sh.packed && gd == CLIPK_F32 && prefix_split_flag(e, kPrefixSplitBwd) != 0;
}

static int attn_split_flag(const clipk_encoder* e) {
  const char* s = getenv("CLIPK_VIT_SPLIT_ATTN");
  return (s ? atoi(s) != 0 : true) && e->split != 0 && e->act == CLIPK_F32 ? CLIPK_ATTN_SPLIT : 0;
}

static int attn_fwd(const clipk_encoder* e, const SeqShape& sh, const void* qkv, void* o, float* lse,
                    hipStream_t st, int pflags = 0) {
  const int W = e->W;
  if (sh.packed)
    return clipk_attention_prefix_fwd_ex(e->act, sh.G, sh.P, sh.R, sh.ntiles, sh.tiles, sh.row_first, e->heads,
                                         qkv, 3 * W, o, W, lse,
                                         pflags | prefix_split_flag(e, kPrefixSplitFwd) |
                                             (t_osplit ? CLIPK_PREFIX_OUT_SPLIT : 0), st);
  return clipk_attention_fwd_ex(e->act, sh.nseq, sh.L, e->heads, sh.causal, qkv, 3 * W, o, W, lse,
                                attn_split_flag(e) | (t_osplit ? CLIPK_ATTN_OUT_SPLIT : 0), st);
}

static int attn_bwd(const clipk_encoder* e, const SeqShape& sh, const void* qkv, const void* o,
                    const void* dout, const float* lse, void* dqkv, void* part, hipStream_t st,
                    bool dqkv_split = false, int pflags = 0) {
  const int W = e->W;
  if (sh.packed)
    return clipk_attention_prefix_bwd_ex(e->act, dqkv_split ? CLIPK_F32S : e->grad, sh.G, sh.P, sh.R, sh.ntiles, sh.tiles, sh.row_first,
                                      e->heads, qkv, 3 * W, o, W, dout, W, lse, dqkv, 3 * W, part,
                                      sh.part_bytes(e->heads),
                                      pflags | (prefix_split_bwd(e, sh, e->grad) ? CLIPK_PREFIX_SPLIT : 0), st);
  return clipk_attention_bwd(e->act, e->grad, sh.nseq, sh.L, e->heads, sh.causal, qkv, 3 * W, o, W, dout, W,
                             lse, dqkv, 3 * W, st);
}

static int block_attn(const clipk_encoder* e, const std::array<const void*, 16>& w, const SeqShape& sh, int rd,
                      const void* X, void* xn, void* qkv, void* o, float* lse, float* m1, float* r1,
                      hipStream_t st, bool text, void* sk, size_t skb) {
  const int pg = text ? CLIPK_PROF_GEMM_ALL : CLIPK_PROF_NONE;
  const int W = e->W, rows = sh.rows, act = e->act;
  const double lnb = (double)rows * W * (esize(rd) + esize(act)) + (m1 ? 8.0 * rows : 0.0);
  {
    ProfScope ps(CLIPK_PROF_NONE, st, 0.0, text ? "text.ln_fwd" : "vit.ln_fwd", lnb);
    TRY(clipk_layernorm_fwd_x(rd, act, rows, W, X, W, nullptr, (const float*)w[0], (const float*)w[1], xn, W,
                              m1, r1, st));
  }
  TRY(gemm(act, act, CLIPK_EPI_BIAS, rows, 3 * W, W, xn, w[2], (const float*)w[3], nullptr, qkv,
           nullptr, nullptr, 0, st, pg, sk, skb, text ? "text.qkv_fwd" : "vit.qkv_fwd"));
  {
    const double ab = (double)rows * 4 * W * esize(act) + (lse ? 4.0 * rows * e->heads : 0.0);
    ProfScope ps(text ? CLIPK_PROF_ATTN : CLIPK_PROF_NONE, st, 0.0, text ? "text.attn_fwd" : "vit.attn_fwd", ab);
    TRY(attn_fwd(e, sh, qkv, o, lse, st));
  }
  return CLIPK_OK;
}


static bool presplit_on() {
  static int v = -1;
  if (v < 0) {
    const char* s = getenv("CLIPK_PRESPLIT");
    v = s ? atoi(s) : 1;
  }
  return v != 0;
}
static int ps_out() { return t_split && presplit_on() ? CLIPK_OUT_SPLIT : 0; }
static int ps_a() { return t_split && presplit_on() ? CLIPK_A_SPLIT : 0; }

static int block_post(const clipk_encoder* e, const std::array<const void*, 16>& w, int rows, int rd,
                      const void* X, const void* o, void* Xm, void* Xo, void* xn, void* h, void* g, float* m2,
                      float* r2, hipStream_t st, bool text, void* sk, size_t skb) {
  const int pg = text ? CLIPK_PROF_GEMM_ALL : CLIPK_PROF_NONE;
  const int W = e->W, act = e->act;
  TRY(gemm(act, rd, CLIPK_EPI_BIAS_RES, rows, W, W, o, w[4], (const float*)w[5], X, Xm,
           nullptr, nullptr, 0, st, pg, sk, skb, text ? "text.out_fwd" : "vit.out_fwd"));
  {
    const double lnb = (double)rows * W * (esize(rd) + esize(act)) + (m2 ? 8.0 * rows : 0.0);
    ProfScope ps(CLIPK_PROF_NONE, st, 0.0, text ? "text.ln_fwd" : "vit.ln_fwd", lnb);
    TRY(clipk_layernorm_fwd_x(rd, act, rows, W, Xm, W, nullptr, (const float*)w[6], (const float*)w[7], xn, W,
                              m2, r2, st));
  }
  const int pso = sk ? 0 : ps_out(), psa = sk ? 0 : ps_a();
  TRY(gemm(act, act, CLIPK_EPI_BIAS_QGELU | (h ? CLIPK_QGELU_DERIV : 0) | pso, rows, 4 * W, W, xn, w[8], (const float*)w[9],
           nullptr, g, h, nullptr, 0, st, text ? CLIPK_PROF_GEMM_FC : CLIPK_PROF_NONE, sk, skb, text ? "text.fc_fwd" : "vit.fc_fwd"));
  TRY(gemm(act, rd, CLIPK_EPI_BIAS_RES | psa, rows, W, 4 * W, g, w[10], (const float*)w[11], Xm, Xo,
           nullptr, nullptr, 0, st, pg, sk, skb, text ? "text.proj_fwd" : "vit.proj_fwd"));
  return CLIPK_OK;
}

static int block_fwd(const clipk_encoder* e, const std::array<const void*, 16>& w, const SeqShape& sh,
                     int rd, const void* X, void* Xm, void* Xo, void* xn, void* qkv, void* o,
                     float* lse, void* h, void* g, float* m1, float* r1, float* m2, float* r2,
                     hipStream_t st, bool text, void* sk = nullptr, size_t skb = 0) {
  TRY(block_attn(e, w, sh, rd, X, xn, qkv, o, lse, m1, r1, st, text, sk, skb));
  return block_post(e, w, sh.rows, rd, X, o, Xm, Xo, xn, h, g, m2, r2, st, text, sk, skb);
}

static int gemm_ln(int act, int epi, int M, int N, int K, const void* A, const void* B, const float* bias,
                   const void* res, void* o, void* o2, float* stats, const float* colsum, const float* rnb,
                   hipStream_t st, int prof_cls, const char* site, const float* gamma = nullptr) {
  const double b = gemm_bytes(act, act, epi, M, N, K, o2 != nullptr, act) + (stats ? (double)M * (N / 64) * 8 : 0.0) +
                   (rnb ? 8.0 * M : 0.0) + (gamma ? 4.0 * K : 0.0);
  ProfScope ps(prof_cls, st, 2.0 * M * N * K, site, b);
  if (t_split && act == CLIPK_F32) act = t_split == 2 ? CLIPK_F32S16 : CLIPK_F32S;
  if (gamma) return clipk_gemm_ln_gamma(act, epi, M, N, K, A, K, B, K, bias, o, N, o2, colsum, rnb, gamma, st);
  return clipk_gemm_ln(act, epi, M, N, K, A, K, B, K, bias, res, N, o, N, o2, stats, colsum, rnb, st);
}
static int gemm_ln_split2(int epi, int M, int N, int K, const void* A, const void* B, const float* bias,
                          const void* res, void* o, float* stats, const float* gamma, void* xs, hipStream_t st,
                          int prof_cls, const char* site) {
  const double b = gemm_bytes(CLIPK_F32S16, CLIPK_F32, epi, M, N, K, false, CLIPK_F32) + (double)M * (N / 64) * 8 +
                   4.0 * M * N + 4.0 * N;
  ProfScope ps(prof_cls, st, 2.0 * M * N * K, site, b);
  return clipk_gemm_ln_stats_split(CLIPK_F32S16, epi, M, N, K, A, K, B, K, bias, res, N, o, N, stats, gamma, xs, st);
}
static bool ps_fold(const clipk_encoder* e) { return t_split == 2 && e->split == 2 && presplit_on(); }
static bool o_split_on(const clipk_encoder* e, const SeqShape& sh, bool fold) {
  const char* s = getenv("CLIPK_PRESPLIT_O");
  return (s ? atoi(s) != 0 : true) && fold && ps_fold(e) && sh.packed && e->lora.rank == 0 &&
         prefix_split_flag(e, kPrefixSplitFwd) != 0 && prefix_split_bwd(e, sh, e->grad);
}
static bool vit_o_split_on(const clipk_encoder* e, const SeqShape& sh, bool fold, bool save) {
  const char* s = getenv("CLIPK_PRESPLIT_O");
  return (s ? atoi(s) != 0 : true) && !save && fold && ps_fold(e) && !sh.packed && sh.L > 16 && e->lora.rank == 0 &&
         attn_split_flag(e) != 0;
}
static int ln_merge(int rows, int W, const float* lnst, float* m, float* r, float* rnb, hipStream_t st, bool text) {
  ProfScope ps(CLIPK_PROF_NONE, st, 0.0, text ? "text.ln_stats" : "vit.ln_stats", (double)rows * (W / 64) * 8 + 16.0 * rows);
  return clipk_ln_stats_merge(rows, W, lnst, m, r, rnb, st);
}
static int gemm_ln_merged(int act, int epi, int M, int N, int K, const void* A, const void* B, const float* bias,
                          void* o, void* o2, const float* lnst, const float* colsum, float* m, float* r,
                          float* rnb, hipStream_t st, int prof_cls, const char* site, bool text,
                          const float* gamma = nullptr) {
  if (t_split || act == CLIPK_F32 || !clipk_gemm_ln_merge_fused(act, M, N, K)) {
    TRY(ln_merge(M, K, lnst, m, r, rnb, st, text));
    return gemm_ln(act, epi, M, N, K, A, B, bias, nullptr, o, o2, nullptr, colsum, rnb, st, prof_cls, site, gamma);
  }
  const double b = gemm_bytes(act, act, epi, M, N, K, o2 != nullptr, act) + (double)M * (K / 64) * 8 + 16.0 * M;
  ProfScope ps(prof_cls, st, 2.0 * M * N * K, site, b);
  return clipk_gemm_ln_merge(act, epi, M, N, K, A, K, B, K, bias, o, N, o2, lnst, colsum, m, r, rnb, st);
}
static int block_attn_fold(const clipk_encoder* e, const std::array<const void*, 6>& f, const SeqShape& sh,
                           const void* X, void* qkv, void* o, float* lse, float* m1, float* r1, const float* lnst,
                           float* rnb, hipStream_t st, bool text, const float* gamma = nullptr,
                           const void* xs = nullptr) {
  const int W = e->W, rows = sh.rows, act = e->act;
  TRY(gemm_ln_merged(act, CLIPK_EPI_BIAS | (xs ? CLIPK_A_SPLIT : 0), rows, 3 * W, W, xs ? xs : X, f[0],
                     (const float*)f[2], qkv, nullptr, lnst, (const float*)f[1], m1, r1, rnb, st,
                     text ? CLIPK_PROF_GEMM_ALL : CLIPK_PROF_NONE, text ? "text.qkv_fwd" : "vit.qkv_fwd", text, gamma));
  const double ab = (double)rows * 4 * W * esize(act) + (lse ? 4.0 * rows * e->heads : 0.0);
  ProfScope ps(text ? CLIPK_PROF_ATTN : CLIPK_PROF_NONE, st, 0.0, text ? "text.attn_fwd" : "vit.attn_fwd", ab);
  return attn_fwd(e, sh, qkv, o, lse, st);
}
static int block_post_fold(const clipk_encoder* e, const std::array<const void*, 16>& w,
                           const std::array<const void*, 6>& f, int rows, const void* X, const void* o, void* Xm,
                           void* Xo, void* h, void* g, float* m2, float* r2, float* lnst, float* rnb,
                           bool stats_next, hipStream_t st, bool text, void* xs = nullptr,
                           const float* gamma_next = nullptr) {
  const int W = e->W, act = e->act;
  const int pg = text ? CLIPK_PROF_GEMM_ALL : CLIPK_PROF_NONE;
  const float* g2 = e->split == 2 ? (const float*)w[6] : nullptr;
  if (xs)
    TRY(gemm_ln_split2(CLIPK_EPI_BIAS_RES | (t_osplit ? CLIPK_A_SPLIT : 0), rows, W, W, o, w[4], (const float*)w[5], X,
                       Xm, lnst, g2, xs, st, pg, text ? "text.out_fwd" : "vit.out_fwd"));
  else if (t_osplit)
    return CLIPK_EINVAL;
  else
    TRY(gemm_ln(act, CLIPK_EPI_BIAS_RES, rows, W, W, o, w[4], (const float*)w[5], X, Xm, nullptr, lnst, nullptr,
                nullptr, st, pg, text ? "text.out_fwd" : "vit.out_fwd"));
  TRY(gemm_ln_merged(act, CLIPK_EPI_BIAS_QGELU | (h ? CLIPK_QGELU_DERIV : 0) | ps_out() |
                              (xs ? CLIPK_A_SPLIT : 0),
                     rows, 4 * W, W, xs ? xs : Xm, f[3], (const float*)f[5], g, h, lnst, (const float*)f[4], m2, r2,
                     rnb, st, text ? CLIPK_PROF_GEMM_FC : CLIPK_PROF_NONE, text ? "text.fc_fwd" : "vit.fc_fwd", text,
                     g2));
  if (stats_next && xs && gamma_next)
    return gemm_ln_split2(CLIPK_EPI_BIAS_RES | ps_a(), rows, W, 4 * W, g, w[10], (const float*)w[11], Xm, Xo, lnst,
                          gamma_next, xs, st, pg, text ? "text.proj_fwd" : "vit.proj_fwd");
  if (stats_next)
    return gemm_ln(act, CLIPK_EPI_BIAS_RES | ps_a(), rows, W, 4 * W, g, w[10], (const float*)w[11], Xm, Xo, nullptr,
                   lnst, nullptr, nullptr, st, pg, text ? "text.proj_fwd" : "vit.proj_fwd");
  return gemm(act, act, CLIPK_EPI_BIAS_RES | ps_a(), rows, W, 4 * W, g, w[10], (const float*)w[11], Xm, Xo, nullptr,
              nullptr, 0, st, pg, nullptr, 0, text ? "text.proj_fwd" : "vit.proj_fwd");
}

}

using namespace clipk;

extern "C" const char* clipk_strerror(int status) {
  switch (status) {
    case CLIPK_OK: return "ok";
    case CLIPK_EINVAL: return "invalid argument (null pointer or bad enum)";
    case CLIPK_ESHAPE: return "shape violates a kernel constraint";
    case CLIPK_EDTYPE: return "unsupported dtype combination";
    case CLIPK_EWORKSPACE: return "workspace too small";
    case CLIPK_ERANGE: return "input outside the supported range (clipk_split_pack: |W| >= 65504 / 64 or not finite; clipk_split_hi16: W not fp16-valued)";
    case CLIPK_EHIP: return "a HIP runtime call of a synchronous check failed";
    default: return status > 0 ? hipGetErrorString((hipError_t)status) : "unknown error";
  }
}

extern "C" int clipk_device_arch_ok(void) {
  hipDeviceProp_t p;
  if (hipGetDeviceProperties(&p, 0) != hipSuccess) return 0;
  return std::strncmp(p.gcnArchName, "gfx950", 6) == 0 ? 1 : 0;
}

extern "C" int clipk_encoder_create(int width, int layers, int heads, int embed, int act_dtype,
                                    int grad_dtype, const void* const* layer_ptrs,
                                    const void* const* head_ptrs, clipk_encoder** out) {
  if (!layer_ptrs || !head_ptrs || !out) return CLIPK_EINVAL;
  if (width <= 0 || width % 128 || layers <= 0 || heads * 64 != width || embed % 128 || embed <= 0)
    return CLIPK_ESHAPE;
  if (act_dtype < 0 || act_dtype > 2 || grad_dtype < 0 || grad_dtype > 2) return CLIPK_EDTYPE;
  auto* e = new (std::nothrow) clipk_encoder();
  if (!e) return CLIPK_EINVAL;
  e->kind = 0; e->W = width; e->layers = layers; e->heads = heads; e->E = embed;
  e->act = act_dtype; e->grad = grad_dtype; e->res = e->patch = e->Kp = e->Limg = 0;
  e->lw.resize(layers);
  for (int l = 0; l < layers; ++l)
    for (int i = 0; i < 16; ++i) e->lw[l][i] = layer_ptrs[l * 16 + i];
  for (int i = 0; i < 4; ++i) e->head[i] = head_ptrs[i];
  for (int i = 4; i < 8; ++i) e->head[i] = nullptr;
  *out = e;
  return CLIPK_OK;
}

extern "C" int clipk_vision_create(int width, int layers, int heads, int embed, int res, int patch,
                                   int act_dtype, const void* const* layer_ptrs,
                                   const void* const* head_ptrs, clipk_encoder** out) {
  if (!layer_ptrs || !head_ptrs || !out) return CLIPK_EINVAL;
  if (width <= 0 || width % 128 || layers <= 0 || heads * 64 != width || embed % 128 || patch <= 0 ||
      res % patch)
    return CLIPK_ESHAPE;
  auto* e = new (std::nothrow) clipk_encoder();
  if (!e) return CLIPK_EINVAL;
  e->kind = 1; e->W = width; e->layers = layers; e->heads = heads; e->E = embed;
  e->act = act_dtype; e->grad = act_dtype; e->res = res; e->patch = patch;
  const int k = 3 * patch * patch;
  const int kq = act_dtype == CLIPK_F32 ? 32 : 64;
  e->Kp = (k + kq - 1) / kq * kq;
  e->Limg = (res / patch) * (res / patch) + 1;
  e->lw.resize(layers);
  for (int l = 0; l < layers; ++l)
    for (int i = 0; i < 16; ++i) e->lw[l][i] = layer_ptrs[l * 16 + i];
  for (int i = 0; i < 8; ++i) e->head[i] = head_ptrs[i];
  *out = e;
  return CLIPK_OK;
}

extern "C" void clipk_encoder_destroy(clipk_encoder* enc) { delete enc; }

namespace clipk {

static bool text_eot_last(const SeqShape& sh) {
  static int v = -1;
  if (v < 0) {
    const char* s = getenv("CLIPK_TEXT_EOT_LAST");
    v = s ? atoi(s) : 1;
  }
  return v != 0 && sh.nout < sh.rows;
}

struct EncIO {
  int rd;
  const float *lnf_w, *lnf_b;
  const void* proj_f;
  const void* proj_b;
  bool text;
  void* sk = nullptr;
  size_t skb = 0;
};
static EncIO text_io(const clipk_encoder* e) {
  EncIO io;
  io.rd = res_dtype(e);
  io.lnf_w = (const float*)e->head[0]; io.lnf_b = (const float*)e->head[1];
  io.proj_f = e->head[2]; io.proj_b = e->head[3];
  io.text = true;
  return io;
}
#define SITE(n) (io.text ? "text." n : "vit." n)

static bool ln_fold_on(const clipk_encoder* e, const EncIO& io) {
  static int v = -1;
  if (v < 0) {
    const char* s = getenv("CLIPK_TEXT_LNFOLD");
    v = s ? atoi(s) : 1;
  }
  return v != 0 && (int)e->fold.size() == e->layers && (e->act != CLIPK_F32 || e->split) && io.rd == e->act &&
         e->W % 128 == 0 && e->W <= 1024 && !(e->deep.n_deep > 0 && e->deep.prompts);
}

static int deep_inject(const clipk_encoder* e, int l, int rd, void* X, hipStream_t st) {
  const DeepPrompts& d = e->deep;
  if (l < 1 || l > d.n_deep || !d.prompts) return CLIPK_OK;
  return clipk_rows_inject(rd, d.n_ctx, d.n_per, e->W, d.prompts + (size_t)(l - 1) * d.n_ctx * e->W, d.rows, X,
                           e->W, st);
}

static bool prefix_mode(const clipk_encoder* e, const SeqShape& sh) {
  return e->prefix_input && sh.packed && sh.P >= 1 && sh.R - sh.P >= sh.G * sh.P;
}
__global__ __launch_bounds__(256) void prefix_tables_kernel(int G, int P, int R, int shared, int* __restrict__ prow,
                                                            const float* __restrict__ m, const float* __restrict__ r,
                                                            float* __restrict__ mc, float* __restrict__ rc) {
  const int i = blockIdx.x * 256 + threadIdx.x;
  if (i >= G * P) return;
  const int g = i / P, p = i % P;
  prow[i] = g * R + p;
  if (m) {
    const int si = (!shared || g == 0) ? g * R + p : R + (g - 1) * P + p;
    mc[i] = m[si];
    rc[i] = r[si];
  }
}
__global__ __launch_bounds__(256) void group_bcast_kernel(int G, int P, int R, int chunks, uint4* __restrict__ buf) {
  const long per = (long)(R - P) * chunks;
  for (long j = (long)blockIdx.x * 256 + threadIdx.x; j < per; j += (long)gridDim.x * 256) {
    const uint4 v = buf[(long)P * chunks + j];
    for (int g = 1; g < G; ++g) buf[(long)g * R * chunks + (long)P * chunks + j] = v;
  }
}
static int prefix_tables(const SeqShape& sh, bool shared, int* prow, const float* m, const float* r, float* mc,
                         float* rc, hipStream_t st) {
  const int n = sh.G * sh.P;
  hipLaunchKernelGGL(prefix_tables_kernel, dim3((n + 255) / 256), dim3(256), 0, st, sh.G, sh.P, sh.R, (int)shared, prow,
                     m, r, mc, rc);
  CLIPK_CHECK_LAUNCH();
  return CLIPK_OK;
}

static bool share0_index_on() {
  static int v = -1;
  if (v < 0) {
    const char* s = getenv("CLIPK_SHARE0_INDEX");
    v = s ? atoi(s) : 1;
  }
  return v != 0;
}
static int block_attn_shared0(const clipk_encoder* e, const std::array<const void*, 16>& w, const SeqShape& sh,
                              int rd, const void* X, void* xn, void* qkv, void* o, float* lse, float* m1, float* r1,
                              int* prow, hipStream_t st) {
  const int W = e->W, act = e->act, G = sh.G, P = sh.P, R = sh.R;
  const int n = (G - 1) * P;
  const size_t xa = (size_t)W * esize(act), qa = 3 * xa;
  TRY(prefix_tables(sh, true, prow, nullptr, nullptr, nullptr, nullptr, st));
  {
    ProfScope ps(CLIPK_PROF_NONE, st, 0.0, "text.ln_fwd", (double)(R + n) * W * (esize(rd) + esize(act)));
    TRY(clipk_layernorm_fwd_x(rd, act, R, W, X, W, nullptr, (const float*)w[0], (const float*)w[1], xn, W, m1, r1,
                              st));
    TRY(clipk_layernorm_fwd_x(rd, act, n, W, X, W, prow + P, (const float*)w[0], (const float*)w[1],
                              (char*)xn + (size_t)R * xa, W, m1 ? m1 + R : nullptr, r1 ? r1 + R : nullptr, st));
  }
  TRY(gemm(act, act, CLIPK_EPI_BIAS, R + n, 3 * W, W, xn, w[2], (const float*)w[3], nullptr, qkv, nullptr, nullptr,
           0, st, CLIPK_PROF_GEMM_ALL, nullptr, 0, "text.qkv_fwd"));
  {
    ProfScope ps(CLIPK_PROF_NONE, st, 0.0, "text.qkv_bcast",
                 (double)(G - 2 > 0 ? G - 2 : 0) * P * qa * 2.0 + (share0_index_on() ? 0.0 : (double)(G - 1) * (R - P) * qa * 2.0));
    if (G > 2) TRY(clipk_rows_copy((int)qa, (G - 2) * P, (char*)qkv + (size_t)(R + P) * qa, nullptr, qkv, prow + 2 * P, st));
    if (!share0_index_on()) {
      const int chunks = (int)(qa / 16);
      const long total = (long)(R - P) * chunks;
      hipLaunchKernelGGL(group_bcast_kernel, dim3((unsigned)std::min<long>((total + 255) / 256, 4096)), dim3(256), 0,
                         st, G, P, R, chunks, (uint4*)qkv);
      CLIPK_CHECK_LAUNCH();
    }
  }
  {
    const double ab = (double)sh.rows * 4 * W * esize(act) + (lse ? 4.0 * sh.rows * e->heads : 0.0);
    ProfScope ps(CLIPK_PROF_ATTN, st, 0.0, "text.attn_fwd", ab);
    TRY(attn_fwd(e, sh, qkv, o, lse, st, share0_index_on() ? CLIPK_PREFIX_CLS_GROUP0 : 0));
  }
  return CLIPK_OK;
}

static int text_forward_impl(const clipk_encoder* e, const SeqShape& sh, const float* x0, const int* eot_rows,
                             float* txt, void* saved, size_t saved_bytes, void* ws, size_t ws_bytes,
                             hipStream_t st, const EncIO& io) {
  SplitScope split_scope(e);
  const bool save = saved != nullptr;
  TextBufs t = text_layout(e, sh.rows, sh.nout, saved, ws, save, io.rd);
  if (ws_bytes < t.ws_bytes || (save && saved_bytes < t.saved_bytes)) return CLIPK_EWORKSPACE;
  const int W = e->W, rows = sh.rows, rd = io.rd;
  const int pg = io.text ? CLIPK_PROF_GEMM_ALL : CLIPK_PROF_NONE;
  const void* cur = x0;
  if (save || rd != CLIPK_F32) {
    if (rd == CLIPK_F32) {
      TRY(clipk_rows_copy(W * 4, rows, x0, nullptr, t.X[0], nullptr, st));
    } else {
      TRY(clipk_cast(rd, (long)rows * W, x0, t.X[0], st));
    }
    cur = t.X[0];
  }
  const bool eotl = text_eot_last(sh);
  const int nl = e->layers, nout = sh.nout;
  const bool fold = ln_fold_on(e, io);
  t_osplit = io.text ? o_split_on(e, sh, fold) : vit_o_split_on(e, sh, fold, save);
  if (save) e->o_saved_split = t_osplit;
  bool have_stats = false;
  bool xs_ready = false;
  for (int l = 0; l < nl; ++l) {
    void* Xo = t.X[l + 1];
    if (!save && Xo == cur) Xo = t.X[l];
    if (l >= 1) TRY(deep_inject(e, l, rd, const_cast<void*>(cur), st));
    const bool share0 = l == 0 && io.text && sh.G >= 2 && prefix_mode(e, sh);
    float* m1 = save ? t.mean1[l] : t.tm;
    float* r1 = save ? t.rstd1[l] : t.tr;
    float* m2 = save ? t.mean2[l] : t.tm;
    float* r2 = save ? t.rstd2[l] : t.tr;
    if (share0)
      TRY(block_attn_shared0(e, e->lw[l], sh, rd, cur, t.xn, t.qkv[l], t.o[l], t.lse[l], t.mean1[l], t.rstd1[l],
                             (int*)t.g, st));
    else if (fold && have_stats)
      TRY(block_attn_fold(e, e->fold[l], sh, cur, t.qkv[l], t.o[l], t.lse[l], m1, r1, t.lnst, t.rnb, st, io.text,
                          e->split == 2 ? (const float*)e->lw[l][0] : nullptr, xs_ready ? t.xn : nullptr));
    else
      TRY(block_attn(e, e->lw[l], sh, rd, cur, t.xn, t.qkv[l], t.o[l], t.lse[l], t.mean1[l], t.rstd1[l], st,
                     io.text, io.sk, io.skb));
    const bool compact = eotl && l == nl - 1;
    const void* xin = cur;
    const void* oin = t.o[l];
    if (compact) {
      ProfScope ps(CLIPK_PROF_NONE, st, 0.0, SITE("eot_gather"), 2.0 * nout * W * (esize(e->act) + esize(rd)));
      TRY(clipk_rows_copy(W * (int)esize(e->act), nout, t.o[l], eot_rows, t.oc, nullptr, st));
      TRY(clipk_rows_copy(W * (int)esize(rd), nout, cur, eot_rows, t.xc, nullptr, st));
      xin = t.xc;
      oin = t.oc;
    }
    const int n = compact ? nout : sh.rows;
    void* xs = fold && ps_fold(e) ? t.xn : nullptr;
    const float* gnext = l + 1 < nl ? (const float*)e->lw[l + 1][0] : nullptr;
    xs_ready = xs && gnext;
    if (fold)
      TRY(block_post_fold(e, e->lw[l], e->fold[l], n, xin, oin, t.Xm[l], Xo, save ? t.h[l] : nullptr, t.g, m2, r2,
                          t.lnst, t.rnb, l + 1 < nl, st, io.text, xs, gnext));
    else
      TRY(block_post(e, e->lw[l], n, rd, xin, oin, t.Xm[l], Xo, t.xn, save ? t.h[l] : nullptr, t.g, t.mean2[l],
                     t.rstd2[l], st, io.text, compact ? nullptr : io.sk, compact ? 0 : io.skb));
    have_stats = fold && l + 1 < nl;
    cur = Xo;
  }
  TRY(clipk_layernorm_fwd_x(rd, e->act, sh.nout, W, cur, W, eotl ? nullptr : eot_rows, io.lnf_w, io.lnf_b, t.lnf, W,
                            t.meanf, t.rstdf, st));
  TRY(gemm(e->act, CLIPK_F32, CLIPK_EPI_NONE, sh.nout, e->E, W, t.lnf, io.proj_f, nullptr, nullptr, txt,
           nullptr, nullptr, 0, st, pg, nullptr, 0, SITE("head")));
  return split_check(e, 1, (long)sh.nout * e->E, 0, txt, 1, st);
}

static bool text_dres16(const clipk_encoder* e) {
  static int v = -2;
  if (v == -2) {
    const char* s = getenv("CLIPK_TEXT_DRES16");
    v = s ? atoi(s) : -1;
  }
  if (e->grad == CLIPK_F32 || v == 0) return false;
  return v > 0 || e->grad == CLIPK_F16;
}

__global__ __launch_bounds__(256) void zero16_kernel(long n, uint4* __restrict__ p) {
  for (long i = (long)blockIdx.x * 256 + threadIdx.x; i < n; i += (long)gridDim.x * 256) p[i] = make_uint4(0, 0, 0, 0);
}
static int zero_bytes(void* p, size_t bytes, hipStream_t st) {
  if (bytes == 0) return CLIPK_OK;
  if ((bytes | (uintptr_t)p) & 15) return CLIPK_ESHAPE;
  const long n = (long)(bytes / 16);
  hipLaunchKernelGGL(zero16_kernel, dim3((unsigned)std::min<long>((n + 255) / 256, 4096)), dim3(256), 0, st, n,
                     (uint4*)p);
  CLIPK_CHECK_LAUNCH();
  return CLIPK_OK;
}

static int text_backward_impl(const clipk_encoder* e, const SeqShape& sh, const int* eot_rows,
                              const float* dtxt, const void* saved, size_t saved_bytes, float* dx0,
                              void* ws, size_t ws_bytes, hipStream_t st, const EncIO& io) {
  SplitScope split_scope(e);
  TextBufs t = text_layout(e, sh.rows, sh.nout, const_cast<void*>(saved), nullptr, true, io.rd);
  TextBwdBufs b = text_bwd_layout(e, sh.rows, sh.nout, sh.part_bytes(e->heads), ws);
  if (saved_bytes < t.saved_bytes || ws_bytes < b.bytes) return CLIPK_EWORKSPACE;
  const int W = e->W, rows = sh.rows, nout = sh.nout, gd = e->grad, act = e->act;
  const int pg = io.text ? CLIPK_PROF_GEMM_ALL : CLIPK_PROF_NONE;
  if (e->o_saved_split && !prefix_split_bwd(e, sh, gd)) return CLIPK_EINVAL;
  float* dX = dx0;
  if (e->split) {
    TRY(grad_scale_in(e, (long)nout * e->E, dtxt, (float*)b.dtg, b.gscale, st));
  } else {
    TRY(clipk_cast(gd, (long)nout * e->E, dtxt, b.dtg, st));
  }
  TRY(gemm(gd, CLIPK_F32, CLIPK_EPI_NONE, nout, W, e->E, b.dtg, io.proj_b, nullptr, nullptr, b.dlnf,
           nullptr, nullptr, 0, st, pg));
  const bool r16 = io.rd != CLIPK_F32 && text_dres16(e);
  const bool a_split = e->split == 2 && presplit_on() && !r16 && gd == CLIPK_F32;
  const bool lp_alias = !r16 && gd == CLIPK_F32 && !a_split;
  const int lpd = a_split ? CLIPK_F32S : gd;
  const int dA_split = a_split ? CLIPK_A_SPLIT : 0;
  static const bool qkv_knob = [] {
    const char* s = getenv("CLIPK_PRESPLIT_QKV");
    return s ? atoi(s) != 0 : true;
  }();
  const bool qkv_split = a_split && sh.packed && qkv_knob;
  const int dqkv_split = qkv_split ? CLIPK_A_SPLIT : 0;
  void* const dA = lp_alias ? (void*)dX : b.dX_lp;
  const bool eotl = text_eot_last(sh);
  auto zero = [&](void* p, size_t bytes) { return zero_bytes(p, bytes, st); };
  if (!eotl) {
    if (!r16) TRY(zero(dX, (size_t)rows * W * 4));
    if (!lp_alias) TRY(zero(b.dX_lp, (size_t)rows * W * esize(gd)));
  }
  const int rd = io.rd;
  const int* frows = eotl ? nullptr : eot_rows;
  TRY(clipk_layernorm_bwd_x2(rd, CLIPK_F32, nout, W, b.dlnf, W, t.Xf, W, frows, io.lnf_w, t.meanf,
                             t.rstdf, nullptr, CLIPK_F32, W, r16 ? nullptr : dX, lp_alias ? nullptr : b.dX_lp, lpd,
                             frows, W, st));
  auto ln_bwd = [&](int n, const void* x, const float* gamma, const float* mean, const float* rstd, bool last) {
    const double lnbb = (double)n * W * (esize(gd) + esize(rd) + 2.0 * (r16 ? esize(gd) : 4)) + 8.0 * n;
    ProfScope ps(CLIPK_PROF_NONE, st, 0.0, SITE("ln_bwd"), lnbb);
    if (!r16)
      return clipk_layernorm_bwd_x(rd, gd, n, W, b.dxn, W, x, W, nullptr, gamma, mean, rstd, dX, W, dX,
                                   last || lp_alias ? nullptr : b.dX_lp, lpd, nullptr, W, st);
    return clipk_layernorm_bwd_x2(rd, gd, n, W, b.dxn, W, x, W, nullptr, gamma, mean, rstd, b.dX_lp, gd, W,
                                  last ? dX : nullptr, b.dX_lp, gd, nullptr, W, st);
  };
  const int dgelu_epi = CLIPK_EPI_DQGELU | CLIPK_QGELU_DERIV;
  const clipk_encoder::Lora& lo = e->lora;
  const bool lora_grad = lo.rank > 0 && lo.dA && lo.dB;
  const size_t lora_n = (size_t)3 * lo.rank * W;
  if (lora_grad)
    for (int l = 0; l < e->layers; ++l)
      if (!((lo.layer_mask >> l) & 1u)) {
        TRY(zero(lo.dA + l * lora_n, lora_n * 4));
        TRY(zero(lo.dB + l * lora_n, lora_n * 4));
      }
  for (int l = e->layers - 1; l >= 0; --l) {
    const auto& w = e->lw[l];
    if (!w[12] || !w[13] || !w[14] || !w[15]) return CLIPK_EINVAL;
    const bool compact = eotl && l == e->layers - 1;
    const int n = compact ? nout : rows;
    TRY(gemm(gd, gd, dgelu_epi | ps_out() | dA_split, n, 4 * W, W, dA, w[15], nullptr, nullptr,
             b.dh, nullptr, t.h[l], act, st, io.text ? CLIPK_PROF_GEMM_DGELU : CLIPK_PROF_NONE, nullptr, 0,
             compact ? SITE("proj_dx_dgelu_eot") : SITE("proj_dx_dgelu")));
    TRY(gemm(gd, gd, CLIPK_EPI_NONE | ps_a(), n, W, 4 * W, b.dh, w[14], nullptr, nullptr, b.dxn,
             nullptr, nullptr, 0, st, pg, nullptr, 0, compact ? SITE("fc_dx_eot") : SITE("fc_dx")));
    TRY(ln_bwd(n, t.Xm[l], (const float*)w[6], t.mean2[l], t.rstd2[l], false));
    TRY(gemm(gd, gd, CLIPK_EPI_NONE | dA_split, n, W, W, dA, w[13], nullptr, nullptr, compact ? b.dh : b.do_,
             nullptr, nullptr, 0, st, pg, nullptr, 0, compact ? SITE("out_dx_eot") : SITE("out_dx")));
    if (compact) {
      const int gb = W * (int)esize(gd), rb = W * (r16 ? (int)esize(gd) : 4);
      void* res = r16 ? b.dX_lp : (void*)dX;
      ProfScope ps(CLIPK_PROF_NONE, st, 0.0, SITE("eot_scatter"),
                   2.0 * nout * (gb + 2.0 * rb) + (double)rows * (gb + rb));
      TRY(zero(b.do_, (size_t)rows * gb));
      TRY(clipk_rows_copy(gb, nout, b.dh, nullptr, b.do_, eot_rows, st));
      TRY(clipk_rows_copy(rb, nout, res, nullptr, b.dqkv, nullptr, st));
      TRY(zero(res, (size_t)rows * rb));
      TRY(clipk_rows_copy(rb, nout, b.dqkv, nullptr, res, eot_rows, st));
    }
    {
      const bool reads_o = act == CLIPK_F32 && !prefix_split_bwd(e, sh, gd);
      const double ab = (double)rows * W * ((reads_o ? 4.0 : 3.0) * esize(act) + 4.0 * esize(gd)) +
                        4.0 * rows * e->heads;
      ProfScope ps(io.text ? CLIPK_PROF_ATTN : CLIPK_PROF_NONE, st, 0.0, SITE("attn_bwd"), ab);
      const bool shared0 = l == 0 && io.text && sh.G >= 2 && prefix_mode(e, sh) && share0_index_on();
      TRY(attn_bwd(e, sh, t.qkv[l], t.o[l], b.do_, t.lse[l], b.dqkv, b.part, st, qkv_split,
                   shared0 ? CLIPK_PREFIX_CLS_GROUP0 : 0));
    }
    if (lora_grad && ((lo.layer_mask >> l) & 1u)) {
      ProfScope ps(CLIPK_PROF_NONE, st, 0.0, SITE("lora_wgrad"), 2.0 * rows * W * (esize(rd) + 3.0 * esize(gd)));
      TRY(clipk_lora_wgrad(rd, gd, rows, W, lo.rank, lo.proj_mask, lo.scale, t.X[l], t.mean1[l], t.rstd1[l],
                           (const float*)w[0], (const float*)w[1], b.dqkv, lo.A + l * lora_n, lo.B + l * lora_n,
                           lo.dA + l * lora_n, lo.dB + l * lora_n, b.lora, b.lora_bytes, st));
    }
    if (l == 0 && io.text && prefix_mode(e, sh)) {
      const int np = sh.G * sh.P;
      int* prow = (int*)b.do_;
      float* mc = (float*)(prow + np);
      float* rc = mc + np;
      TRY(prefix_tables(sh, sh.G >= 2, prow, t.mean1[0], t.rstd1[0], mc, rc, st));
      TRY(clipk_rows_copy(3 * W * (int)esize(gd), np, b.dqkv, prow, b.dh, nullptr, st));
      TRY(gemm(gd, gd, CLIPK_EPI_NONE | dqkv_split, np, W, 3 * W, b.dh, w[12], nullptr, nullptr, b.dxn, nullptr,
               nullptr, 0, st, pg, nullptr, 0, SITE("qkv_dx_prefix")));
      const float* g0 = (const float*)w[0];
      if (!r16)
        TRY(clipk_layernorm_bwd_x(rd, gd, np, W, b.dxn, W, t.X[0], W, prow, g0, mc, rc, dX, W, dX, nullptr, gd, prow,
                                  W, st));
      else
        TRY(clipk_layernorm_bwd_x2(rd, gd, np, W, b.dxn, W, t.X[0], W, prow, g0, mc, rc, b.dX_lp, gd, W, dX, b.dX_lp,
                                   gd, prow, W, st));
      continue;
    }
    TRY(gemm(gd, gd, CLIPK_EPI_NONE | dqkv_split, rows, W, 3 * W, b.dqkv, w[12], nullptr, nullptr, b.dxn,
             nullptr, nullptr, 0, st, pg, nullptr, 0, SITE("qkv_dx")));
    TRY(ln_bwd(rows, t.X[l], (const float*)w[0], t.mean1[l], t.rstd1[l], l == 0));
    const DeepPrompts& d = e->deep;
    if (l >= 1 && l <= d.n_deep && d.grads) {
      if (r16)
        TRY(clipk_rows_collect(gd, d.n_ctx, d.n_per, W, b.dX_lp, W, nullptr, 0, 0, d.rows,
                               d.grads + (size_t)(l - 1) * d.n_ctx * W, 0, 1, st));
      else
        TRY(clipk_rows_collect(CLIPK_F32, d.n_ctx, d.n_per, W, dX, W, lp_alias ? nullptr : b.dX_lp, gd, W, d.rows,
                               d.grads + (size_t)(l - 1) * d.n_ctx * W, 0, 1, st));
    }
  }
  if (e->split) {
    TRY(grad_scale_out((long)rows * W, dX, b.gscale, st));
    const DeepPrompts& d = e->deep;
    if (d.n_deep > 0 && d.grads) TRY(grad_scale_out((long)d.n_deep * d.n_ctx * W, d.grads, b.gscale, st));
    if (lora_grad) {
      TRY(grad_scale_out((long)(e->layers * lora_n), lo.dA, b.gscale, st));
      TRY(grad_scale_out((long)(e->layers * lora_n), lo.dB, b.gscale, st));
    }
    if (io.text && prefix_mode(e, sh))
      TRY(split_check(e, sh.G, (long)sh.P * W, (long)sh.R * W, dX, 2, st));
    else
      TRY(split_check(e, 1, (long)rows * W, 0, dX, 2, st));
    if (d.n_deep > 0 && d.grads) TRY(split_check(e, 1, (long)d.n_deep * d.n_ctx * W, 0, d.grads, 2, st));
    if (lora_grad) {
      TRY(split_check(e, 1, (long)(e->layers * lora_n), 0, lo.dA, 2, st));
      TRY(split_check(e, 1, (long)(e->layers * lora_n), 0, lo.dB, 2, st));
    }
  }
  return CLIPK_OK;
}

static size_t text_ws_bytes(const clipk_encoder* e, size_t rows, int nout) {
  TextBufs a = text_layout(e, rows, nout, nullptr, nullptr, true);
  TextBufs b = text_layout(e, rows, nout, nullptr, nullptr, false);
  return a.ws_bytes > b.ws_bytes ? a.ws_bytes : b.ws_bytes;
}

}

extern "C" size_t clipk_text_saved_bytes(const clipk_encoder* e, int nseq, int L) {
  if (!e || nseq <= 0 || L <= 0) return 0;
  return text_layout(e, (size_t)nseq * L, nseq, nullptr, nullptr, true).saved_bytes;
}

extern "C" size_t clipk_text_ws_bytes(const clipk_encoder* e, int nseq, int L) {
  if (!e || nseq <= 0 || L <= 0) return 0;
  return text_ws_bytes(e, (size_t)nseq * L, nseq);
}

extern "C" int clipk_text_forward(const clipk_encoder* e, int nseq, int L, const float* x0,
                                  const int* eot_rows, float* txt, void* saved, size_t saved_bytes,
                                  void* ws, size_t ws_bytes, void* stream) {
  if (!e || e->kind != 0 || !x0 || !eot_rows || !txt || !ws) return CLIPK_EINVAL;
  if (nseq <= 0 || L <= 0 || L > 77) return CLIPK_ESHAPE;
  return text_forward_impl(e, SeqShape::plain(nseq, L, 1), x0, eot_rows, txt, saved, saved_bytes, ws,
                           ws_bytes, (hipStream_t)stream, text_io(e));
}

extern "C" size_t clipk_text_bwd_ws_bytes(const clipk_encoder* e, int nseq, int L) {
  if (!e || nseq <= 0 || L <= 0) return 0;
  return text_bwd_layout(e, (size_t)nseq * L, nseq, 0, nullptr).bytes;
}

extern "C" int clipk_text_backward(const clipk_encoder* e, int nseq, int L, const int* eot_rows,
                                   const float* dtxt, const void* saved, size_t saved_bytes, float* dx0,
                                   void* ws, size_t ws_bytes, void* stream) {
  if (!e || e->kind != 0 || !eot_rows || !dtxt || !saved || !dx0 || !ws) return CLIPK_EINVAL;
  if (!e->head[3]) return CLIPK_EINVAL;
  if (nseq <= 0 || L <= 0 || L > 77) return CLIPK_ESHAPE;
  return text_backward_impl(e, SeqShape::plain(nseq, L, 1), eot_rows, dtxt, saved, saved_bytes, dx0, ws,
                            ws_bytes, (hipStream_t)stream, text_io(e));
}

static bool packed_ok(int G, int C, int P, int R, int ntiles) {
  return G > 0 && C > 0 && P >= 1 && P <= 16 && ntiles >= 1 && R >= P + C && (long)G * R < (1L << 31);
}

extern "C" size_t clipk_text_packed_saved_bytes(const clipk_encoder* e, int G, int C, int R) {
  if (!e || G <= 0 || C <= 0 || R <= 0) return 0;
  return text_layout(e, (size_t)G * R, G * C, nullptr, nullptr, true).saved_bytes;
}

extern "C" size_t clipk_text_packed_ws_bytes(const clipk_encoder* e, int G, int C, int R) {
  if (!e || G <= 0 || C <= 0 || R <= 0) return 0;
  return text_ws_bytes(e, (size_t)G * R, G * C);
}

extern "C" size_t clipk_text_packed_bwd_ws_bytes(const clipk_encoder* e, int G, int C, int R, int ntiles) {
  if (!e || G <= 0 || C <= 0 || R <= 0 || ntiles <= 0) return 0;
  return text_bwd_layout(e, (size_t)G * R, G * C, clipk_attention_prefix_ws_bytes(G, ntiles, e->heads), nullptr)
      .bytes;
}

extern "C" int clipk_text_forward_packed(const clipk_encoder* e, int G, int C, int P, int R, int ntiles,
                                         const int* tiles, const int* row_first, const float* x0,
                                         const int* eot_rows, float* txt, void* saved, size_t saved_bytes,
                                         void* ws, size_t ws_bytes, void* stream) {
  if (!e || e->kind != 0 || !tiles || !row_first || !x0 || !eot_rows || !txt || !ws) return CLIPK_EINVAL;
  if (!packed_ok(G, C, P, R, ntiles)) return CLIPK_ESHAPE;
  if (e->lora.rank > 0) return CLIPK_EINVAL;
  return text_forward_impl(e, SeqShape::prefix(G, C, P, R, ntiles, tiles, row_first), x0, eot_rows, txt, saved,
                           saved_bytes, ws, ws_bytes, (hipStream_t)stream, text_io(e));
}

extern "C" int clipk_text_backward_packed(const clipk_encoder* e, int G, int C, int P, int R, int ntiles,
                                          const int* tiles, const int* row_first, const int* eot_rows,
                                          const float* dtxt, const void* saved, size_t saved_bytes,
                                          float* dx0, void* ws, size_t ws_bytes, void* stream) {
  if (!e || e->kind != 0 || !tiles || !row_first || !eot_rows || !dtxt || !saved || !dx0 || !ws)
    return CLIPK_EINVAL;
  if (!e->head[3]) return CLIPK_EINVAL;
  if (!packed_ok(G, C, P, R, ntiles)) return CLIPK_ESHAPE;
  if (e->lora.rank > 0) return CLIPK_EINVAL;
  return text_backward_impl(e, SeqShape::prefix(G, C, P, R, ntiles, tiles, row_first), eot_rows, dtxt, saved,
                            saved_bytes, dx0, ws, ws_bytes, (hipStream_t)stream, text_io(e));
}

namespace clipk {
struct VitBufs {
  void *patches, *xn, *qkv, *o, *g, *cls;
  float *pout, *x0, *x1, *xm;
  void* sk;
  size_t sk_bytes, bytes;
};
static VitBufs vit_layout(const clipk_encoder* e, int B, void* ws) {
  VitBufs v;
  const size_t a = esize(e->act), D = e->W, L = e->Limg, rows = (size_t)B * L;
  const size_t np = (size_t)B * (L - 1);
  Carver c(ws);
  v.patches = c.take(np * e->Kp * a);
  v.pout = (float*)c.take(np * D * 4);
  v.x0 = (float*)c.take(rows * D * 4);
  v.x1 = (float*)c.take(rows * D * 4);
  v.xm = (float*)c.take(rows * D * 4);
  v.xn = c.take(rows * D * a);
  v.qkv = c.take(rows * 3 * D * a);
  v.o = c.take(rows * D * a);
  v.g = c.take(rows * 4 * D * a);
  v.cls = c.take((size_t)B * D * a);
  static const bool no_sk = getenv("CLIPK_VIT_NOSPLITK") != nullptr;
  v.sk_bytes = no_sk ? 0 : vit_splitk_bytes(e->act, (int)rows, (int)D);
  v.sk = v.sk_bytes ? c.take(v.sk_bytes) : nullptr;
  v.bytes = c.off;
  return v;
}
}

namespace clipk {
static bool vit_res16(const clipk_encoder* e);
static size_t vit16_bytes(const clipk_encoder* e, int B, void* ws, void** parts);
static int vit16_forward(const clipk_encoder* e, int B, const float* img, float* feat, void* ws, size_t ws_bytes,
                         hipStream_t st);
}

extern "C" size_t clipk_vit_ws_bytes(const clipk_encoder* e, int B) {
  if (!e || e->kind != 1) return 0;
  if (vit_res16(e)) return vit16_bytes(e, B, nullptr, nullptr);
  return vit_layout(e, B, nullptr).bytes;
}

extern "C" int clipk_vit_forward(const clipk_encoder* e, int B, const float* img, float* feat,
                                 void* ws, size_t ws_bytes, void* stream) {
  if (!e || e->kind != 1 || !img || !feat || !ws) return CLIPK_EINVAL;
  if (B <= 0) return CLIPK_ESHAPE;
  if (vit_res16(e)) return vit16_forward(e, B, img, feat, ws, ws_bytes, (hipStream_t)stream);
  SplitScope split_scope(e);
  VitBufs v = vit_layout(e, B, ws);
  if (ws_bytes < v.bytes) return CLIPK_EWORKSPACE;
  hipStream_t st = (hipStream_t)stream;
  const int D = e->W, L = e->Limg, np = B * (L - 1), act = e->act;
  TRY(clipk_im2col(act, B, e->res, e->patch, e->Kp, img, v.patches, st));
  TRY(gemm(act, CLIPK_F32, CLIPK_EPI_NONE, np, D, e->Kp, v.patches, e->head[5], nullptr, nullptr,
           v.pout, nullptr, nullptr, 0, st, CLIPK_PROF_NONE,
           clipk_gemm_splitk_ws_bytes(np, D, clipk_gemm_auto_splits(act, np, D, e->Kp)) <= v.sk_bytes ? v.sk : nullptr,
           v.sk_bytes, "vit.patch_embed"));
  TRY(clipk_vit_embed_ln(B, L, D, v.pout, (const float*)e->head[6], (const float*)e->head[7],
                         (const float*)e->head[0], (const float*)e->head[1], v.x0, st));
  float* cur = v.x0;
  float* nxt = v.x1;
  for (int l = 0; l < e->layers; ++l) {
    TRY(block_fwd(e, e->lw[l], SeqShape::plain(B, L, 0), CLIPK_F32, cur, v.xm, nxt, v.xn, v.qkv, v.o, nullptr, nullptr, v.g,
                  nullptr, nullptr, nullptr, nullptr, st, false, v.sk, v.sk_bytes));
    float* t = cur; cur = nxt; nxt = t;
  }
  TRY(clipk_layernorm_fwd(act, B, D, cur, L * D, nullptr, (const float*)e->head[2],
                          (const float*)e->head[3], v.cls, D, nullptr, nullptr, st));
  TRY(gemm(act, CLIPK_F32, CLIPK_EPI_NONE, B, e->E, D, v.cls, e->head[4], nullptr, nullptr, feat,
           nullptr, nullptr, 0, st, CLIPK_PROF_NONE, nullptr, 0, "vit.head"));
  return split_check(e, 1, (long)B * e->E, 0, feat, 1, st);
}

namespace clipk {
static EncIO vit_io(const clipk_encoder* e, const void* proj_b) {
  EncIO io;
  io.rd = CLIPK_F32;
  io.lnf_w = (const float*)e->head[2]; io.lnf_b = (const float*)e->head[3];
  io.proj_f = e->head[4]; io.proj_b = proj_b;
  io.text = false;
  return io;
}
struct VitPBufs {
  void* patches;
  float *pout, *x0, *cls_rows;
  float *dvpt_sum, *vmean, *vrstd;
  void* sk;
  size_t sk_bytes;
  void* rest;
  size_t bytes;
};
static VitPBufs vitp_layout(const clipk_encoder* e, int B, int n_vpt, void* ws) {
  VitPBufs v;
  const size_t a = esize(e->act), D = e->W, L = e->Limg, Lp = L + n_vpt, rows = (size_t)B * Lp;
  const size_t np = (size_t)B * (L - 1);
  Carver c(ws);
  v.patches = c.take(np * e->Kp * a);
  v.pout = (float*)c.take(np * D * 4);
  v.x0 = (float*)c.take(rows * D * 4);
  v.cls_rows = (float*)c.take((size_t)B * 4);
  v.dvpt_sum = (float*)c.take((size_t)(n_vpt > 0 ? n_vpt : 1) * D * 4);
  v.vmean = (float*)c.take((size_t)(n_vpt > 0 ? n_vpt : 1) * 4);
  v.vrstd = (float*)c.take((size_t)(n_vpt > 0 ? n_vpt : 1) * 4);
  static const bool no_sk = getenv("CLIPK_VIT_NOSPLITK") != nullptr;
  v.sk_bytes = no_sk ? 0 : vit_splitk_bytes(e->act, (int)rows, (int)D);
  v.sk = v.sk_bytes ? c.take(v.sk_bytes) : nullptr;
  v.rest = ws ? (char*)ws + c.off : nullptr;
  const size_t fwd = text_layout(e, rows, B, nullptr, nullptr, true, CLIPK_F32).ws_bytes;
  const size_t fwd0 = text_layout(e, rows, B, nullptr, nullptr, false, CLIPK_F32).ws_bytes;
  const size_t bwd = text_bwd_layout(e, rows, B, 0, nullptr).bytes;
  v.bytes = c.off + std::max(std::max(fwd, fwd0), bwd);
  return v;
}
__global__ void cls_rows_kernel(int B, int Lp, int* rows) {
  const int b = blockIdx.x * blockDim.x + threadIdx.x;
  if (b < B) rows[b] = b * Lp;
}

static bool vit_res16(const clipk_encoder* e) {
  static int v = -1, v32 = -1;
  if (v < 0) {
    const char* s = getenv("CLIPK_VIT_RES16");
    v = s ? atoi(s) : 1;
    const char* s32 = getenv("CLIPK_VIT_LOOP32");
    v32 = s32 ? atoi(s32) : 1;
  }
  if (e->act == CLIPK_F32) return v32 != 0 && e->split != 0;
  return v != 0;
}
static size_t vit16_bytes(const clipk_encoder* e, int B, void* ws, void** parts) {
  const size_t a = esize(e->act), D = e->W, L = e->Limg, rows = (size_t)B * L;
  const size_t np = (size_t)B * (L - 1);
  Carver c(ws);
  void* p[6];
  p[0] = c.take(np * e->Kp * a);
  p[1] = c.take(np * D * 4);
  p[2] = c.take(rows * D * 4);
  p[3] = c.take((size_t)B * 4);
  static const bool no_sk = getenv("CLIPK_VIT_NOSPLITK") != nullptr;
  const size_t skb = no_sk ? 0 : vit_splitk_bytes(e->act, (int)rows, (int)D);
  p[4] = skb ? c.take(skb) : nullptr;
  p[5] = ws ? (char*)ws + c.off : nullptr;
  if (parts)
    for (int i = 0; i < 6; ++i) parts[i] = p[i];
  return c.off + text_layout(e, rows, B, nullptr, nullptr, false, e->act).ws_bytes;
}
static int vit16_forward(const clipk_encoder* e, int B, const float* img, float* feat, void* ws, size_t ws_bytes,
                         hipStream_t st) {
  void* p[6];
  const size_t need = vit16_bytes(e, B, ws, p);
  if (ws_bytes < need) return CLIPK_EWORKSPACE;
  SplitScope split_scope(e);
  const int D = e->W, L = e->Limg, np = B * (L - 1), act = e->act;
  const size_t skb = p[4] ? (size_t)((char*)p[5] - (char*)p[4]) : 0;
  TRY(clipk_im2col(act, B, e->res, e->patch, e->Kp, img, p[0], st));
  TRY(gemm(act, CLIPK_F32, CLIPK_EPI_NONE, np, D, e->Kp, p[0], e->head[5], nullptr, nullptr, p[1], nullptr, nullptr,
           0, st, CLIPK_PROF_NONE,
// ... 218 lines not shown
```

### include/clipk.h

```cpp
#ifndef CLIPK_H
#define CLIPK_H

#include <stddef.h>
#include <stdint.h>

#ifdef __cplusplus
extern "C" {
#endif

enum { CLIPK_F32 = 0, CLIPK_F16 = 1, CLIPK_BF16 = 2, CLIPK_F32S = 3, CLIPK_F32S16 = 4 };

enum {
  CLIPK_OK = 0,
  CLIPK_EINVAL = -1,
  CLIPK_ESHAPE = -2,
  CLIPK_EDTYPE = -3,
  CLIPK_EWORKSPACE = -4,
  CLIPK_ERANGE = -5,
  CLIPK_EHIP = -6
};

enum {
  CLIPK_EPI_BIAS = 0,
  CLIPK_EPI_BIAS_RES = 1,
  CLIPK_EPI_BIAS_QGELU = 2,
  CLIPK_EPI_DQGELU = 3,
  CLIPK_EPI_NONE = 4
};
enum { CLIPK_A_QGELU = 0x100 };
enum { CLIPK_QGELU_DERIV = 0x200 };
enum { CLIPK_OUT_SPLIT = 0x400, CLIPK_A_SPLIT = 0x800, CLIPK_OUT2_SPLIT_GAMMA = 0x1000 };

const char* clipk_version(void);
const char* clipk_source_digest(void);
const char* clipk_strerror(int status);
int clipk_device_arch_ok(void);

int clipk_gemm(int in_dtype, int out_dtype, int epi, int M, int N, int K,
               const void* A, int lda, const void* B, int ldb,
               const float* bias, const void* res, int ldr,
               void* out, int ldo, void* out2, const void* aux, int aux_dtype, int ldaux,
               void* stream);

#define CLIPK_SPLIT_SCALE 64.0f
int clipk_split_pack(int N, int K, const float* W, int ldw, void* out, void* stream);
int clipk_split_lo_zero(int N, int K, const void* packed, int* result, void* stream);
int clipk_split_hi16(int N, int K, const void* packed, void* out, void* stream);

int clipk_gemm_auto_splits(int in_dtype, int M, int N, int K);
size_t clipk_gemm_splitk_ws_bytes(int M, int N, int splits);
int clipk_gemm_splitk(int in_dtype, int out_dtype, int epi, int M, int N, int K,
                      const void* A, int lda, const void* B, int ldb,
                      const float* bias, const void* res, int ldr,
                      void* out, int ldo, void* out2, int splits, void* ws, size_t ws_bytes,
                      void* stream);

int clipk_gemm_ln_gamma(int in_dtype, int epi, int M, int N, int K, const void* A, int lda, const void* B, int ldb,
                        const float* bias, void* out, int ldo, void* out2, const float* colsum, const float* rnb,
                        const float* gamma, void* stream);
int clipk_gemm_ln(int in_dtype, int epi, int M, int N, int K, const void* A, int lda, const void* B, int ldb,
                  const float* bias, const void* res, int ldr, void* out, int ldo, void* out2,
                  float* stats, const float* colsum, const float* rnb, void* stream);
int clipk_gemm_ln_stats_split(int in_dtype, int epi, int M, int N, int K, const void* A, int lda, const void* B,
                              int ldb, const float* bias, const void* res, int ldr, void* out, int ldo, float* stats,
                              const float* gamma, void* out2, void* stream);
int clipk_ln_stats_merge(int rows, int width, const float* stats, float* mean, float* rstd, float* rnb,
                         void* stream);
int clipk_gemm_ln_merge(int in_dtype, int epi, int M, int N, int K, const void* A, int lda, const void* B,
                        int ldb, const float* bias, void* out, int ldo, void* out2, const float* stats,
                        const float* colsum, float* mean, float* rstd, float* rnb, void* stream);
int clipk_gemm_ln_merge_fused(int in_dtype, int M, int N, int K);
int clipk_gemm_split_tile_rows(int in_dtype, int epi, int lnm, int M, int N);
double clipk_gemm_t256_cost(int in_dtype, int epi, int lnm);
int clipk_gemm_set_config(int cfg);

int clipk_image_resample(int B, int S, int rows_max, const void* src, const long long* desc,
                         const int* tables, void* tmp, const float* mean, const float* stdv,
                         int out_uint8, void* out, void* stream);

enum { CLIPK_COLOR_BRIGHTNESS = 1, CLIPK_COLOR_CONTRAST = 2, CLIPK_COLOR_SATURATION = 3,
       CLIPK_COLOR_HUE = 4, CLIPK_COLOR_GRAYSCALE = 5 };
enum { CLIPK_COLOR_MAX_OPS = 5, CLIPK_COLOR_DESC = 12 };
int clipk_image_color(int B, int S, void* pix, const int* prog, int* prog_dev, const float* mean,
                      const float* stdv, int out_uint8, void* out, void* stream);

int clipk_gemm_stamps(void* host, size_t bytes);

int clipk_vit_embed_ln_vpt(int B, int L, int n_vpt, int width, const float* patch, const float* cls,
                           const float* pos, const float* vpt, const float* gamma, const float* beta, float* x,
                           void* stream);

int clipk_rows_inject(int dst_dtype, int n_ctx, int n_per, int width, const float* src, const int* rows,
                      void* dst, int ldd, void* stream);
int clipk_rows_collect(int src_dtype, int n_ctx, int n_per, int width, void* src, int lds, void* src2,
                       int src2_dtype, int lds2, const int* rows, float* out, int accumulate, int zero_src,
                       void* stream);

int clipk_layernorm_fwd(int out_dtype, int rows, int width, const float* x, int ldx,
                        const int* in_rows, const float* gamma, const float* beta,
                        void* out, int ldo, float* mean, float* rstd, void* stream);
int clipk_layernorm_fwd_x(int x_dtype, int out_dtype, int rows, int width, const void* x, int ldx,
                          const int* in_rows, const float* gamma, const float* beta,
                          void* out, int ldo, float* mean, float* rstd, void* stream);

int clipk_layernorm_bwd(int dy_dtype, int rows, int width, const void* dy, int lddy, const float* x, int ldx,
                        const int* x_rows, const float* gamma, const float* mean, const float* rstd,
                        const float* dres, int lddres, float* dx, void* dx_lp, int lp_dtype,
                        const int* out_rows, int ldo, void* stream);
int clipk_layernorm_bwd_x(int x_dtype, int dy_dtype, int rows, int width, const void* dy, int lddy,
                          const void* x, int ldx, const int* x_rows, const float* gamma,
                          const float* mean, const float* rstd, const float* dres, int lddres,
                          float* dx, void* dx_lp, int lp_dtype, const int* out_rows, int ldo,
                          void* stream);
int clipk_layernorm_bwd_x2(int x_dtype, int dy_dtype, int rows, int width, const void* dy, int lddy,
                           const void* x, int ldx, const int* x_rows, const float* gamma,
                           const float* mean, const float* rstd, const void* dres, int dres_dtype,
                           int lddres, float* dx, void* dx_lp, int lp_dtype, const int* out_rows,
                           int ldo, void* stream);

int clipk_attention_fwd(int dtype, int nseq, int L, int heads, int causal,
                        const void* qkv, int ldqkv, void* out, int ldo, float* lse, void* stream);
enum { CLIPK_ATTN_SPLIT = 1, CLIPK_ATTN_OUT_SPLIT = 2 };
int clipk_attention_fwd_ex(int dtype, int nseq, int L, int heads, int causal,
                           const void* qkv, int ldqkv, void* out, int ldo, float* lse, int flags,
                           void* stream);

int clipk_attention_bwd(int dtype, int grad_dtype, int nseq, int L, int heads, int causal,
                        const void* qkv, int ldqkv, const void* ofwd, int ldof, const void* dout,
                        int lddo, const float* lse, void* dqkv, int lddqkv, void* stream);

int clipk_attention_prefix_fwd(int dtype, int G, int P, int R, int ntiles, const int* tiles,
                               const int* row_first, int heads, const void* qkv, int ldqkv, void* out,
                               int ldo, float* lse, void* stream);
size_t clipk_attention_prefix_ws_bytes(int G, int ntiles, int heads);
int clipk_attention_prefix_bwd(int dtype, int grad_dtype, int G, int P, int R, int ntiles,
                               const int* tiles, const int* row_first, int heads, const void* qkv,
                               int ldqkv, const void* ofwd, int ldof, const void* dout, int lddo,
                               const float* lse, void* dqkv, int lddqkv, void* ws, size_t ws_bytes,
                               void* stream);

enum { CLIPK_PREFIX_CLS_GROUP0 = 1, CLIPK_PREFIX_SPLIT = 2, CLIPK_PREFIX_OUT_SPLIT = 4 };
int clipk_attention_prefix_fwd_ex(int dtype, int G, int P, int R, int ntiles, const int* tiles,
                                  const int* row_first, int heads, const void* qkv, int ldqkv, void* out,
                                  int ldo, float* lse, int flags, void* stream);
int clipk_attention_prefix_bwd_ex(int dtype, int grad_dtype, int G, int P, int R, int ntiles,
                                  const int* tiles, const int* row_first, int heads, const void* qkv,
                                  int ldqkv, const void* ofwd, int ldof, const void* dout, int lddo,
                                  const float* lse, void* dqkv, int lddqkv, void* ws, size_t ws_bytes,
                                  int flags, void* stream);

int clipk_im2col(int out_dtype, int B, int res, int patch, int Kp, const float* img, void* out,
                 void* stream);

int clipk_vit_embed_ln(int B, int L, int width, const float* patch, const float* cls,
                       const float* pos, const float* gamma, const float* beta, float* x,
                       void* stream);

int clipk_prompt_assemble(int B, int C, int L, int W, const int* src_map, const float* emb,
                          const float* ctx, long ctx_sb, long ctx_sc, const float* bias,
                          const float* pos, float* x0, void* stream);

int clipk_ctx_grad(int B, int C, int L, int W, int n_ctx, int csc, const int* ctx_pos,
                   const float* dx0, float* dctx, void* stream);

int clipk_prompt_assemble_rows(int G, int R, int C, int L, int W, const int* row_tab,
                               const int* src_map, const float* emb, const float* ctx, long ctx_sg,
                               long ctx_sc, const float* bias, const float* pos, float* x0,
                               void* stream);
int clipk_ctx_grad_rows(int G, int R, int W, int n_ctx, const int* slot_ptr, const int* slot_rows,
                        const float* dx0, float* dctx, void* stream);

int clipk_ctx_bias_grad_rows(int G, int R, int W, int n_ctx, const int* slot_ptr, const int* slot_rows,
                             const float* dx0, float* dctx, float* dbias, void* stream);

int clipk_cosine_logits_fwd(int B, int C, int E, int per_image, float scale, const float* imf,
                            const float* txt, float* logits, float* inv_tnorm, float* inv_inorm,
                            void* stream);
int clipk_cosine_logits_bwd(int B, int C, int E, int per_image, float scale, const float* imf,
                            const float* txt, const float* inv_tnorm, const float* inv_inorm,
                            const float* dlogits, float* dtxt, void* stream);

int clipk_ce_loss(int B, int C, const float* logits, const int64_t* labels, const float* alpha,
                  float gamma, int focal, float grad_scale, float* row_loss, float* dlogits,
                  void* stream);

int clipk_ce_loss_reduce(int B, int C, const float* logits, const int64_t* labels, const float* alpha,
                         float gamma, int focal, float grad_scale, int reduction, float* row_loss,
                         float* loss, float* dlogits, void* stream);

int clipk_mixup_images(int B, long n_per, const float* x, const int* perm, const int64_t* labels,
                       int64_t* y_b, float w0, float w1, float* out, void* stream);

int clipk_ce_loss_mix(int B, int C, const float* logits, const int64_t* y_a, const int64_t* y_b,
                      float lam, const float* alpha, float gamma, int focal, float grad_scale,
                      int reduction, float* row_loss, float* loss, float* dlogits, void* stream);

size_t clipk_ntxent_ws_bytes(int n, int D);
int clipk_ntxent_loss(int n, int D, const float* a, const float* b, float temperature,
                      float grad_scale, float* loss, float* da, float* db,
                      void* ws, void* stream);

size_t clipk_src_head_ws_bytes(int B, int C, int E);
int clipk_src_head(int B, int C, int E, const float* img, const float* txt, const float* zs_img,
                   const float* fixed_n, const float* fixed_q, const int64_t* labels,
                   const float* alpha, float gamma, int focal, float scale, float w_text,
                   float w_image, float w_logits, float grad_scale, float* loss, float* logits,
                   float* d_img, float* d_txt, void* ws, void* stream);

size_t clipk_probe_head_ws_bytes(int B, int C, int E);
int clipk_probe_head(int B, int C, int E, const float* feat, const float* w, const float* bias,
                     const int64_t* labels, const float* alpha, float gamma, int focal,
                     int normalize, float scale, float grad_scale,
                     float* loss, float* logits, float* d_w, float* d_bias,
                     void* ws, void* stream);

int clipk_meta_net_fwd(int B, int V, int Hd, int Wd, const float* x, const float* w1,
                       const float* b1, const float* w2, const float* b2, float* h, float* y,
                       void* stream);
int clipk_meta_net_fwd_norm(int B, int V, int Hd, int Wd, const float* x, const float* w1,
                            const float* b1, const float* w2, const float* b2, float* xn, float* h,
                            float* y, void* stream);
int clipk_meta_net_bwd(int B, int V, int Hd, int Wd, const float* x, const float* h,
                       const float* w2, const float* dy, float* dw1, float* db1, float* dw2,
                       float* db2, float* dh_ws, void* stream);

int clipk_sgd_step(long n, float* p, const float* g, float* buf, float lr, float momentum,
                   float weight_decay, int has_buf, void* stream);
int clipk_sgd_step_multi(int count, float* const* p, const float* const* g, float* const* buf,
                         const long* n, const int* has_buf, float lr, float momentum,
                         float weight_decay, void* stream);

int clipk_sgd_step_multi_scaled(int count, float* const* p, const float* const* g, float* const* buf,
                                const long* n, const int* has_buf, float lr, float momentum,
                                float weight_decay, float grad_scale, void* stream);
int clipk_sgd_step_multi_if(int count, float* const* p, const float* const* g, float* const* buf,
                            const long* n, const int* has_buf, float lr, float momentum,
                            float weight_decay, float grad_scale, const int* guard, int mask, void* stream);

enum { CLIPK_ADAM_ADAM = 0, CLIPK_ADAM_ADAMW = 1, CLIPK_ADAM_AMSGRAD = 2 };
int clipk_adam_step_multi(int count, float* const* p, const float* const* g, float* const* m,
                          float* const* v, float* const* vmax, const long* n, int* const* step,
                          const int* parity, double lr, double beta1, double beta2, double eps,
                          double weight_decay, int mode, float grad_scale, const int* guard, int mask,
                          void* stream);
int clipk_status_take(int* flags, int* host_word, void* stream);

int clipk_rows_copy(int row_bytes, int n, const void* src, const int* src_rows, void* dst,
                    const int* dst_rows, void* stream);

int clipk_cast(int out_dtype, long n, const float* x, void* y, void* stream);

typedef struct clipk_encoder clipk_encoder;

int clipk_encoder_create(int width, int layers, int heads, int embed, int act_dtype,
                         int grad_dtype, const void* const* layer_ptrs, const void* const* head_ptrs,
                         clipk_encoder** out);
void clipk_encoder_destroy(clipk_encoder* enc);

int clipk_encoder_set_deep_prompts(clipk_encoder* e, int n_deep, int n_ctx, int n_per, const int* rows,
                                   const float* prompts, float* grads);

int clipk_encoder_set_input_rows(clipk_encoder* e, int mode);

int clipk_encoder_set_ln_fold(clipk_encoder* e, const void* const* fold_ptrs);

int clipk_encoder_set_split(clipk_encoder* e, int on);
int clipk_encoder_set_split_target(clipk_encoder* e, int target);
int clipk_encoder_set_status(clipk_encoder* e, int* status);

int clipk_lora_merge(int W, int layers, int rank, int proj_mask, unsigned layer_mask, float scale,
                     int act_dtype, int grad_dtype, const float* const* w0, const float* A, const float* B,
                     void* const* out, void* const* outT, void* stream);
size_t clipk_lora_wgrad_ws_bytes(int rows, int W, int rank);
int clipk_lora_wgrad(int x_dtype, int g_dtype, int rows, int W, int rank, int proj_mask, float scale,
                     const void* X, const float* mean, const float* rstd, const float* gamma,
                     const float* beta, const void* dqkv, const float* A, const float* B, float* dA,
                     float* dB, void* ws, size_t ws_bytes, void* stream);
int clipk_encoder_set_lora(clipk_encoder* e, int rank, int proj_mask, unsigned layer_mask, float scale,
                           const float* A, const float* B, float* dA, float* dB);

size_t clipk_vit_prompted_saved_bytes(const clipk_encoder* e, int B, int n_vpt);
size_t clipk_vit_prompted_ws_bytes(const clipk_encoder* e, int B, int n_vpt);
int clipk_vit_forward_prompted(const clipk_encoder* e, int B, const float* img, int n_vpt, const float* vpt,
                               float* feat, void* saved, size_t saved_bytes, void* ws, size_t ws_bytes,
                               void* stream);
int clipk_vit_backward_prompted(const clipk_encoder* e, int B, int n_vpt, const float* vpt, const void* proj_bwd,
                                const float* dfeat, const void* saved, size_t saved_bytes, float* dvpt, void* ws,
                                size_t ws_bytes, void* stream);

size_t clipk_text_saved_bytes(const clipk_encoder* enc, int nseq, int L);
size_t clipk_text_ws_bytes(const clipk_encoder* enc, int nseq, int L);
int clipk_text_forward(const clipk_encoder* enc, int nseq, int L, const float* x0, const int* eot_rows,
                       float* txt, void* saved, size_t saved_bytes, void* ws, size_t ws_bytes,
                       void* stream);
size_t clipk_text_bwd_ws_bytes(const clipk_encoder* enc, int nseq, int L);
int clipk_text_backward(const clipk_encoder* enc, int nseq, int L, const int* eot_rows,
                        const float* dtxt, const void* saved, size_t saved_bytes, float* dx0,
                        void* ws, size_t ws_bytes, void* stream);

size_t clipk_text_packed_saved_bytes(const clipk_encoder* enc, int G, int C, int R);
size_t clipk_text_packed_ws_bytes(const clipk_encoder* enc, int G, int C, int R);
size_t clipk_text_packed_bwd_ws_bytes(const clipk_encoder* enc, int G, int C, int R, int ntiles);
int clipk_text_forward_packed(const clipk_encoder* enc, int G, int C, int P, int R, int ntiles,
                              const int* tiles, const int* row_first, const float* x0,
                              const int* eot_rows, float* txt, void* saved, size_t saved_bytes,
                              void* ws, size_t ws_bytes, void* stream);
int clipk_text_backward_packed(const clipk_encoder* enc, int G, int C, int P, int R, int ntiles,
                               const int* tiles, const int* row_first, const int* eot_rows,
                               const float* dtxt, const void* saved, size_t saved_bytes, float* dx0,
                               void* ws, size_t ws_bytes, void* stream);

int clipk_vision_create(int width, int layers, int heads, int embed, int res, int patch,
                        int act_dtype, const void* const* layer_ptrs,
                        const void* const* head_ptrs, clipk_encoder** out);
size_t clipk_vit_ws_bytes(const clipk_encoder* enc, int B);
int clipk_vit_forward(const clipk_encoder* enc, int B, const float* img, float* feat, void* ws,
                      size_t ws_bytes, void* stream);

enum { CLIPK_CONV_RES = 1, CLIPK_CONV_RELU = 2, CLIPK_CONV_OUT_F32 = 4 };
int clipk_conv2d_nhwc(int dtype, int flags, int B, int H, int W, int Cin, int Cout, int ksize,
                      const void* x, const void* w, const float* scale, const float* shift,
                      const void* res, void* out, void* stream);
int clipk_im2col_3x3s2(int out_dtype, int B, int res, const float* img, void* out, void* stream);
int clipk_avgpool2_nhwc(int dtype, int B, int H, int W, int C, const void* x, void* out, void* stream);
size_t clipk_attnpool_ws_bytes(int dtype, int B, int HW, int C);
int clipk_attnpool(int dtype, int B, int HW, int C, int heads, int E, const void* x, const float* pos,
                   const void* q_w, const float* q_b, const void* kv_w, const float* kv_b,
                   const void* c_w, const float* c_b, float* feat, void* ws, size_t ws_bytes,
                   void* stream);
typedef struct clipk_resnet clipk_resnet;
int clipk_resnet_create(int width, const int* blocks, int embed, int res, int act_dtype,
                        const void* const* ptrs, int n_ptrs, clipk_resnet** out);
void clipk_resnet_destroy(clipk_resnet* h);
size_t clipk_resnet_ws_bytes(const clipk_resnet* h, int B);
int clipk_resnet_forward(const clipk_resnet* h, int B, const float* img, float* feat, void* ws,
                         size_t ws_bytes, void* stream);

enum { CLIPK_PROF_NONE = 0, CLIPK_PROF_GEMM_FC = 1, CLIPK_PROF_GEMM_ALL = 2, CLIPK_PROF_ATTN = 3,
       CLIPK_PROF_LN = 4, CLIPK_PROF_GEMM_DGELU = 5 };
int clipk_prof_enable(int kind);
int clipk_prof_read(double* total_ms, long* count, double* flops_or_bytes);

enum { CLIPK_PROF_NAME_LEN = 32 };
int clipk_prof_sites_enable(int on);
int clipk_prof_sites_read(int max_sites, char* names, double* total_ms, long* count, double* flops,
                          double* bytes, int* n_sites);

#ifdef __cplusplus
}
#endif
#endif
```

Before: 386.2.

## Restrict text-encoder edge layers to EOT queries and prefix-only gradients

Adds two prefix-attention modes. In the last text layer only the EOT query rows are computed in forward and backward, because only those rows feed the output. In the first layer's backward, query and output gradients are skipped for non-prefix rows, and only the shared prefix rows of x0 are saved instead of copying the whole input. This cuts MFMA work, memory traffic and a full-row copy in the text encoder. In exchange it adds kernel template variants, a column-zeroing kernel and tighter preconditions tying the forward save state to the backward pass.

```diff
diff --git a/few-shot-prompt-learning-for-vision-language-models-in-imbalanced-datasets_amd/_native.py b/few-shot-prompt-learning-for-vision-language-models-in-imbalanced-datasets_amd/_native.py
--- a/few-shot-prompt-learning-for-vision-language-models-in-imbalanced-datasets_amd/_native.py
+++ b/few-shot-prompt-learning-for-vision-language-models-in-imbalanced-datasets_amd/_native.py
@@ -28,6 +28,8 @@
 PREFIX_CLS_GROUP0 = 1
 PREFIX_SPLIT = 2
 PREFIX_OUT_SPLIT = 4
+PREFIX_GRAD_PREFIX = 8
+PREFIX_EOT_QUERIES = 16
 ATTN_SPLIT = 1
 ATTN_OUT_SPLIT = 2
 F32S16 = 4
diff --git a/few-shot-prompt-learning-for-vision-language-models-in-imbalanced-datasets_amd/csrc/attention_prefix.hip b/few-shot-prompt-learning-for-vision-language-models-in-imbalanced-datasets_amd/csrc/attention_prefix.hip
--- a/few-shot-prompt-learning-for-vision-language-models-in-imbalanced-datasets_amd/csrc/attention_prefix.hip
+++ b/few-shot-prompt-learning-for-vision-language-models-in-imbalanced-datasets_amd/csrc/attention_prefix.hip
@@ -1024,7 +1024,13 @@
 }
 constexpr int kSplitFwdWpc = 12, kSplitBwdWpc = 8;
 
-template <int WPB, bool OS>
+__device__ __forceinline__ bool eot_row(const int* __restrict__ row_first, int t0, int n, int r16) {
+  if (r16 >= n) return false;
+  if (r16 == n - 1) return true;
+  return row_first[t0 + r16 + 1] != row_first[t0 + r16];
+}
+
+template <int WPB, bool OS, bool EQ = false>
 __global__ __launch_bounds__(WPB * 64) void attn_prefix_fwd_split(
     int G, int P, int R, int ntiles, const int* __restrict__ tiles, const int* __restrict__ row_first, int H,
     int nchunk, int uc, const float* __restrict__ qkv, int ldq, float* __restrict__ out, int ldo,
@@ -1043,21 +1049,28 @@
   const size_t gR = (size_t)g * R;
   const float* qh = qkv + h * 64 + 4 * g4;
   const int u_begin = k * uc, u_end = min((k + 1) * uc, ntiles + 1);
+  const int u_first = EQ ? max(u_begin, 1) : u_begin;
   const int tab = load_tile_table(tiles, ntiles, u_begin, lane);
 
   f32x4 qn[4], kn[4], vn[4];
   int firstn = 0;
+  bool seln = true;
   auto fetch = [&](int u) {
     int t0, n, pre;
     tile_info(tab, P, u, u_begin, t0, n, pre);
     const int rl = t0 + min(r16, n - 1);
     const float* qp = qh + ((cls0 && u > 0 ? 0 : gR) + rl) * ldq;
-    ld_frag32(qp, qn);
+    if constexpr (EQ) {
+      seln = eot_row(row_first, t0, n, r16);
+      ld_frag32(qp + (seln ? 0 : (long)(t0 + n - 1 - rl) * ldq), qn);
+    } else {
+      ld_frag32(qp, qn);
+    }
     ld_frag32(qp + W, kn);
     ld_frag32(qp + 2 * W, vn);
     firstn = u == 0 ? 0 : row_first[rl] - t0;
   };
-  if (u_begin < u_end) fetch(u_begin);
+  if (u_first < u_end) fetch(u_first);
   Parts8 kp;
   {
     const bool pok = r16 < P;
@@ -1067,14 +1080,19 @@
     ld_prefix_parts(pp + 2 * W, pok, vp);
     st_parts(vp, sVpH, sVpL, r16, g4);
   }
-  for (int u = u_begin; u < u_end; ++u) {
+  for (int u = u_first; u < u_end; ++u) {
     int t0, n, pre;
     tile_info(tab, P, u, u_begin, t0, n, pre);
     const int first = firstn;
-    const bool qok = r16 < n;
+    const bool qok = EQ ? seln : r16 < n;
     Parts8 q, ko;
     {
       Parts8 vo;
+      if constexpr (EQ) {
+#pragma unroll
+        for (int i = 0; i < 4; ++i)
+          if (!qok) qn[i] = (f32x4){0.f, 0.f, 0.f, 0.f};
+      }
       split_frag(qn, q);
       split_frag(kn, ko);
       split_frag(vn, vo);
@@ -1119,7 +1137,7 @@
   }
 }
 
-template <int WPB, bool OS>
+template <int WPB, bool OS, bool PO = false, bool EQ = false>
 __global__ __launch_bounds__(WPB * 64, 2) void attn_prefix_bwd_split(
     int G, int P, int R, int ntiles, const int* __restrict__ tiles, const int* __restrict__ row_first, int H,
     int nchunk, int uc, const float* __restrict__ qkv, int ldq, const float* __restrict__ dout, int lddo,
@@ -1144,24 +1162,32 @@
   const float* dh = dout + h * 64 + 4 * g4;
   const float* lse_h = lse + h;
   const int u_begin = k * uc, u_end = min((k + 1) * uc, ntiles + 1);
+  const int u_first = EQ ? max(u_begin, 1) : u_begin;
   const int tab = load_tile_table(tiles, ntiles, u_begin, lane);
 
   f32x4 qn[4], kn[4], vn[4], dn[4];
   float l2n = 0.f;
   int first2n = 0;
+  constexpr int kNotEot = 0x100;
   auto fetch = [&](int u) {
     int t0, n, pre;
     tile_info(tab, P, u, u_begin, t0, n, pre);
     const int rl = t0 + min(r16, n - 1);
     const float* qp = qh + ((cls0 && u > 0 ? 0 : gR) + rl) * ldq;
-    ld_frag32(qp, qn);
+    int rq = rl;
+    bool sel = true;
+    if constexpr (EQ) {
+      sel = eot_row(row_first, t0, n, r16);
+      rq = sel ? rl : t0 + n - 1;
+    }
+    ld_frag32(qp + (long)(rq - rl) * ldq, qn);
     ld_frag32(qp + W, kn);
     ld_frag32(qp + 2 * W, vn);
-    ld_frag32(dh + (gR + rl) * lddo, dn);
-    l2n = lse_h[(gR + rl) * H];
-    first2n = u == 0 ? 0 : row_first[rl] - t0;
+    ld_frag32(dh + (gR + rq) * lddo, dn);
+    l2n = lse_h[(gR + rq) * H];
+    first2n = (u == 0 ? 0 : row_first[rl] - t0) | (sel ? 0 : kNotEot);
   };
-  if (u_begin < u_end) fetch(u_begin);
+  if (u_first < u_end) fetch(u_first);
   Parts8 kp, vp;
   {
     const bool pok = r16 < P;
@@ -1177,13 +1203,15 @@
     dkp[t] = z;
     dvp[t] = z;
   }
-  for (int u = u_begin; u < u_end; ++u) {
+  for (int u = u_first; u < u_end; ++u) {
     int t0, n, pre;
     tile_info(tab, P, u, u_begin, t0, n, pre);
-    const bool own_is_prefix = u == 0;
+    const bool own_is_prefix = !EQ && u == 0;
+    const bool own_out = !PO || own_is_prefix;
     const bool qok = r16 < n;
+    const bool dq_ok = EQ ? first2n < kNotEot : qok;
     const float l2 = l2n;
-    const int first2 = first2n;
+    const int first2 = EQ ? first2n & (kNotEot - 1) : first2n;
     f32x4 s1p, s2p, p1p, p2p, s1o, s2o, p1o, p2o;
     {
       Parts8 q, ko, vo, d;
@@ -1191,6 +1219,12 @@
       split_frag(kn, ko);
       split_frag(vn, vo);
       split_frag(dn, d);
+      if constexpr (EQ) {
+        if (!dq_ok) {
+          q = Parts8{};
+          d = Parts8{};
+        }
+      }
       lds_fence();
       st_parts(q, tQH, tQL, r16, g4);
       st_parts(ko, tKoH, tKoL, r16, g4);
@@ -1199,9 +1233,11 @@
       s2p = mfma32_s3(kp, q, z);
       p1p = mfma32_s3(d, vp, z);
       p2p = mfma32_s3(vp, d, z);
-      s1o = mfma32_s3(q, ko, z);
+      s1o = z;
+      p1o = z;
+      if (own_out) s1o = mfma32_s3(q, ko, z);
       s2o = mfma32_s3(ko, q, z);
-      p1o = mfma32_s3(d, vo, z);
+      if (own_out) p1o = mfma32_s3(d, vo, z);
       p2o = mfma32_s3(vo, d, z);
     }
     __builtin_amdgcn_sched_barrier(0);
@@ -1240,28 +1276,30 @@
     lds_fence();
     float* orow = dqkv + (gR + t0 + r16) * lddq + h * 64;
     f32x4 acc[4];
-#pragma unroll
-    for (int t = 0; t < 4; ++t) {
-      acc[t] = mfma16_s3(tr_read(tKpH, 4 * g4, 16 * t, lane), tr_read(tKpL, 4 * g4, 16 * t, lane), bTpH, bTpL, z);
-      acc[t] = mfma16_s3(tr_read(tKoH, 4 * g4, 16 * t, lane), tr_read(tKoL, 4 * g4, 16 * t, lane), bToH, bToL, acc[t]);
-    }
-    store_acc64<OS>(orow, acc, kScale, qok, g4);
+    if (own_out) {
+#pragma unroll
+      for (int t = 0; t < 4; ++t) {
+        acc[t] = mfma16_s3(tr_read(tKpH, 4 * g4, 16 * t, lane), tr_read(tKpL, 4 * g4, 16 * t, lane), bTpH, bTpL, z);
+        acc[t] = mfma16_s3(tr_read(tKoH, 4 * g4, 16 * t, lane), tr_read(tKoL, 4 * g4, 16 * t, lane), bToH, bToL, acc[t]);
+      }
+      store_acc64<OS>(orow, acc, kScale, dq_ok, g4);
+    }
 #pragma unroll
     for (int t = 0; t < 4; ++t) {
       const s16x4 aH = tr_read(tQH, 4 * g4, 16 * t, lane), aL = tr_read(tQL, 4 * g4, 16 * t, lane);
       dkp[t] = mfma16_s3(aH, aL, bSpH, bSpL, dkp[t]);
-      acc[t] = mfma16_s3(aH, aL, bSoH, bSoL, z);
+      if (own_out) acc[t] = mfma16_s3(aH, aL, bSoH, bSoL, z);
       if (own_is_prefix) dkp[t] += acc[t];
     }
-    if (!own_is_prefix) store_acc64<OS>(orow + W, acc, kScale, qok, g4);
+    if (!own_is_prefix && own_out) store_acc64<OS>(orow + W, acc, kScale, qok, g4);
 #pragma unroll
     for (int t = 0; t < 4; ++t) {
       const s16x4 aH = tr_read(tDH, 4 * g4, 16 * t, lane), aL = tr_read(tDL, 4 * g4, 16 * t, lane);
       dvp[t] = mfma16_s3(aH, aL, bPpH, bPpL, dvp[t]);
-      acc[t] = mfma16_s3(aH, aL, bPoH, bPoL, z);
+      if (own_out) acc[t] = mfma16_s3(aH, aL, bPoH, bPoL, z);
       if (own_is_prefix) dvp[t] += acc[t];
     }
-    if (!own_is_prefix) store_acc64<OS>(orow + 2 * W, acc, kPInv, qok, g4);
+    if (!own_is_prefix && own_out) store_acc64<OS>(orow + 2 * W, acc, kPInv, qok, g4);
   }
   float* pb = part + ((size_t)g * nchunk + k) * 16 * (2 * W);
   if (r16 < P) {
@@ -1466,22 +1504,27 @@
 
 static int prefix_fwd_split(int G, int P, int R, int ntiles, const int* tiles, const int* row_first, int H,
                             const void* qkv, int ldq, void* out, int ldo, float* lse, hipStream_t st, int cls0,
-                            bool out_split) {
+                            bool out_split, bool eot_q) {
   constexpr int WPB = 4;
   const int uc = f32_uc(G, ntiles, H, kSplitFwdWpc);
   const int nchunk = n_chunks(ntiles, uc);
   const long waves = (long)G * nchunk * H;
-  if (out_split)
-    hipLaunchKernelGGL((attn_prefix_fwd_split<WPB, true>), dim3((waves + WPB - 1) / WPB), dim3(64 * WPB), 0, st, G, P, R,
-                       ntiles, tiles, row_first, H, nchunk, uc, (const float*)qkv, ldq, (float*)out, ldo, lse, cls0);
-  else
-    hipLaunchKernelGGL((attn_prefix_fwd_split<WPB, false>), dim3((waves + WPB - 1) / WPB), dim3(64 * WPB), 0, st, G, P, R,
-                       ntiles, tiles, row_first, H, nchunk, uc, (const float*)qkv, ldq, (float*)out, ldo, lse, cls0);
+  auto go = [&](auto kern) {
+    hipLaunchKernelGGL(kern, dim3((waves + WPB - 1) / WPB), dim3(64 * WPB), 0, st, G, P, R, ntiles, tiles, row_first, H,
+                       nchunk, uc, (const float*)qkv, ldq, (float*)out, ldo, lse, cls0);
+  };
+  if (eot_q) {
+    if (out_split) go(attn_prefix_fwd_split<WPB, true, true>);
+    else go(attn_prefix_fwd_split<WPB, false, true>);
+  } else {
+    if (out_split) go(attn_prefix_fwd_split<WPB, true>);
+    else go(attn_prefix_fwd_split<WPB, false>);
+  }
   CLIPK_CHECK_LAUNCH();
   return CLIPK_OK;
 }
 
-template <bool OS>
+template <bool OS, bool PO = false, bool EQ = false>
 static int prefix_bwd_split(int G, int P, int R, int ntiles, const int* tiles, const int* row_first, int H,
                             const void* qkv, int ldq, const void* dout, int lddo, const float* lse, void* dqkv,
                             int lddq, float* part, hipStream_t st, int cls0) {
@@ -1490,7 +1533,7 @@
   const int uc = f32_uc(G, ntiles, H, kSplitBwdWpc);
   const int nchunk = n_chunks(ntiles, uc);
   const long waves = (long)G * nchunk * H;
-  hipLaunchKernelGGL((attn_prefix_bwd_split<WPB, OS>), dim3((waves + WPB - 1) / WPB), dim3(64 * WPB), 0, st, G, P, R,
+  hipLaunchKernelGGL((attn_prefix_bwd_split<WPB, OS, PO, EQ>), dim3((waves + WPB - 1) / WPB), dim3(64 * WPB), 0, st, G, P, R,
                      ntiles, tiles, row_first, H, nchunk, uc, (const float*)qkv, ldq, (const float*)dout, lddo, lse,
                      (float*)dqkv, lddq, part, cls0);
   CLIPK_CHECK_LAUNCH();
@@ -1522,7 +1565,8 @@
 }
 
 constexpr int kPrefixFlags = CLIPK_PREFIX_CLS_GROUP0 | CLIPK_PREFIX_SPLIT;
-constexpr int kPrefixFwdFlags = kPrefixFlags | CLIPK_PREFIX_OUT_SPLIT;
+constexpr int kPrefixFwdFlags = kPrefixFlags | CLIPK_PREFIX_OUT_SPLIT | CLIPK_PREFIX_EOT_QUERIES;
+constexpr int kPrefixBwdFlags = kPrefixFlags | CLIPK_PREFIX_GRAD_PREFIX | CLIPK_PREFIX_EOT_QUERIES;
 static int prefix_fwd_call(int dtype, int G, int P, int R, int ntiles, const int* tiles, const int* row_first,
                            int heads, const void* qkv, int ldqkv, void* out, int ldo, float* lse, int flags,
                            void* stream) {
@@ -1530,6 +1574,7 @@
   if (flags & ~kPrefixFwdFlags) return CLIPK_EINVAL;
   if ((flags & CLIPK_PREFIX_SPLIT) && dtype != CLIPK_F32) return CLIPK_EINVAL;
   if ((flags & CLIPK_PREFIX_OUT_SPLIT) && (!(flags & CLIPK_PREFIX_SPLIT) || ldo % 8)) return CLIPK_EINVAL;
+  if ((flags & CLIPK_PREFIX_EOT_QUERIES) && !(flags & CLIPK_PREFIX_SPLIT)) return CLIPK_EINVAL;
   if (!prefix_shape_ok(G, P, R, ntiles, heads, ldqkv) || ldqkv < 3 * heads * 64 || ldo < heads * 64 ||
       ldqkv % 8 || ldo % 8)
     return CLIPK_ESHAPE;
@@ -1537,7 +1582,7 @@
   const int c0 = (flags & CLIPK_PREFIX_CLS_GROUP0) ? 1 : 0;
   if (flags & CLIPK_PREFIX_SPLIT)
     return prefix_fwd_split(G, P, R, ntiles, tiles, row_first, heads, qkv, ldqkv, out, ldo, lse, st, c0,
-                            (flags & CLIPK_PREFIX_OUT_SPLIT) != 0);
+                            (flags & CLIPK_PREFIX_OUT_SPLIT) != 0, (flags & CLIPK_PREFIX_EOT_QUERIES) != 0);
   switch (dtype) {
     case CLIPK_F16: return prefix_fwd<f16>(G, P, R, ntiles, tiles, row_first, heads, qkv, ldqkv, out, ldo, lse, st, c0);
     case CLIPK_BF16: return prefix_fwd<bf16>(G, P, R, ntiles, tiles, row_first, heads, qkv, ldqkv, out, ldo, lse, st, c0);
@@ -1563,7 +1608,9 @@
                            const void* dout, int lddo, const float* lse, void* dqkv, int lddqkv, void* ws,
                            size_t ws_bytes, int flags, void* stream) {
   if (!tiles || !row_first || !qkv || !ofwd || !dout || !lse || !dqkv || !ws) return CLIPK_EINVAL;
-  if (flags & ~kPrefixFlags) return CLIPK_EINVAL;
+  if (flags & ~kPrefixBwdFlags) return CLIPK_EINVAL;
+  if ((flags & (CLIPK_PREFIX_GRAD_PREFIX | CLIPK_PREFIX_EOT_QUERIES)) && !(flags & CLIPK_PREFIX_SPLIT))
+    return CLIPK_EINVAL;
   if ((flags & CLIPK_PREFIX_SPLIT) && (dtype != CLIPK_F32 || (grad_dtype != CLIPK_F32 && grad_dtype != CLIPK_F32S)))
     return CLIPK_EINVAL;
   if (!prefix_shape_ok(G, P, R, ntiles, heads, lddqkv) || ldqkv < 3 * heads * 64 || lddqkv < 3 * heads * 64 ||
@@ -1575,13 +1622,22 @@
   const int c0 = (flags & CLIPK_PREFIX_CLS_GROUP0) ? 1 : 0;
   if (flags & CLIPK_PREFIX_SPLIT) {
     if (ldqkv % 4 || lddo % 4 || lddqkv % 4) return CLIPK_ESHAPE;
+    const bool po = (flags & CLIPK_PREFIX_GRAD_PREFIX) != 0, eq = (flags & CLIPK_PREFIX_EOT_QUERIES) != 0;
+    if (grad_dtype == CLIPK_F32S && lddqkv % 8) return CLIPK_ESHAPE;
+#define CLIPK_PBWDS(OS_, PO_, EQ_)                                                                               \
+  return prefix_bwd_split<OS_, PO_, EQ_>(G, P, R, ntiles, tiles, row_first, heads, qkv, ldqkv, dout, lddo, lse, dqkv, \
+                                         lddqkv, part, st, c0)
     if (grad_dtype == CLIPK_F32S) {
-      if (lddqkv % 8) return CLIPK_ESHAPE;
-      return prefix_bwd_split<true>(G, P, R, ntiles, tiles, row_first, heads, qkv, ldqkv, dout, lddo, lse, dqkv,
-                                    lddqkv, part, st, c0);
-    }
-    return prefix_bwd_split<false>(G, P, R, ntiles, tiles, row_first, heads, qkv, ldqkv, dout, lddo, lse, dqkv,
-                                   lddqkv, part, st, c0);
+      if (po && eq) CLIPK_PBWDS(true, true, true);
+      if (po) CLIPK_PBWDS(true, true, false);
+      if (eq) CLIPK_PBWDS(true, false, true);
+      CLIPK_PBWDS(true, false, false);
+    }
+    if (po && eq) CLIPK_PBWDS(false, true, true);
+    if (po) CLIPK_PBWDS(false, true, false);
+    if (eq) CLIPK_PBWDS(false, false, true);
+    CLIPK_PBWDS(false, false, false);
+#undef CLIPK_PBWDS
   }
 #define CLIPK_PBWD(TT, TGG)                                                                           \
   return prefix_bwd<TT, TGG>(G, P, R, ntiles, tiles, row_first, heads, qkv, ldqkv, ofwd, ldof, dout, lddo, \
diff --git a/few-shot-prompt-learning-for-vision-language-models-in-imbalanced-datasets_amd/csrc/encoder.hip b/few-shot-prompt-learning-for-vision-language-models-in-imbalanced-datasets_amd/csrc/encoder.hip
--- a/few-shot-prompt-learning-for-vision-language-models-in-imbalanced-datasets_amd/csrc/encoder.hip
+++ b/few-shot-prompt-learning-for-vision-language-models-in-imbalanced-datasets_amd/csrc/encoder.hip
@@ -34,6 +34,8 @@
     float *dA = nullptr, *dB = nullptr;
   } lora;
   mutable int o_saved_split = 0;
+  mutable bool edge0_saved = false;
+  mutable bool edgeL_saved = false;
 };
 
 namespace clipk {
@@ -477,14 +479,15 @@
 static int block_attn_fold(const clipk_encoder* e, const std::array<const void*, 6>& f, const SeqShape& sh,
                            const void* X, void* qkv, void* o, float* lse, float* m1, float* r1, const float* lnst,
                            float* rnb, hipStream_t st, bool text, const float* gamma = nullptr,
-                           const void* xs = nullptr) {
+                           const void* xs = nullptr, int pflags = 0) {
   const int W = e->W, rows = sh.rows, act = e->act;
   TRY(gemm_ln_merged(act, CLIPK_EPI_BIAS | (xs ? CLIPK_A_SPLIT : 0), rows, 3 * W, W, xs ? xs : X, f[0],
                      (const float*)f[2], qkv, nullptr, lnst, (const float*)f[1], m1, r1, rnb, st,
                      text ? CLIPK_PROF_GEMM_ALL : CLIPK_PROF_NONE, text ? "text.qkv_fwd" : "vit.qkv_fwd", text, gamma));
-  const double ab = (double)rows * 4 * W * esize(act) + (lse ? 4.0 * rows * e->heads : 0.0);
+  const double qrows = (pflags & CLIPK_PREFIX_EOT_QUERIES) ? sh.nout : rows;
+  const double ab = ((double)rows * 2 + qrows * 2) * W * esize(act) + (lse ? 4.0 * qrows * e->heads : 0.0);
   ProfScope ps(text ? CLIPK_PROF_ATTN : CLIPK_PROF_NONE, st, 0.0, text ? "text.attn_fwd" : "vit.attn_fwd", ab);
-  return attn_fwd(e, sh, qkv, o, lse, st);
+  return attn_fwd(e, sh, qkv, o, lse, st, pflags);
 }
 static int block_post_fold(const clipk_encoder* e, const std::array<const void*, 16>& w,
                            const std::array<const void*, 6>& f, int rows, const void* X, const void* o, void* Xm,
@@ -672,6 +675,26 @@
   }
   return v != 0;
 }
+static bool text_edge_rows(const clipk_encoder* e, const SeqShape& sh, const EncIO& io) {
+  static int v = -1;
+  if (v < 0) {
+    const char* s = getenv("CLIPK_TEXT_EDGE_ROWS");
+    v = s ? atoi(s) : 1;
+  }
+  return v != 0 && io.text && io.rd == CLIPK_F32 && e->layers >= 2 && sh.G >= 2 && prefix_mode(e, sh) &&
+         share0_index_on() && prefix_split_bwd(e, sh, e->grad) && text_eot_last(sh) && e->lora.rank == 0 &&
+         !(e->deep.n_deep > 0 && e->deep.prompts);
+}
+static bool text_edge_last(const clipk_encoder* e, const SeqShape& sh, const EncIO& io) {
+  static int v = -1;
+  if (v < 0) {
+    const char* s = getenv("CLIPK_TEXT_EDGE_ROWS");
+    v = s ? atoi(s) : 1;
+  }
+  return v != 0 && io.text && io.rd == CLIPK_F32 && sh.packed && e->layers >= 2 && text_eot_last(sh) &&
+         prefix_split_flag(e, kPrefixSplitFwd) != 0 && prefix_split_bwd(e, sh, e->grad) && e->lora.rank == 0 &&
+         !(e->deep.n_deep > 0 && e->deep.prompts);
+}
 static int block_attn_shared0(const clipk_encoder* e, const std::array<const void*, 16>& w, const SeqShape& sh,
                               int rd, const void* X, void* xn, void* qkv, void* o, float* lse, float* m1, float* r1,
                               int* prow, hipStream_t st) {
@@ -718,7 +741,9 @@
   const int W = e->W, rows = sh.rows, rd = io.rd;
   const int pg = io.text ? CLIPK_PROF_GEMM_ALL : CLIPK_PROF_NONE;
   const void* cur = x0;
-  if (save || rd != CLIPK_F32) {
+  const bool edge0 = save && text_edge_rows(e, sh, io);
+  if (save) e->edge0_saved = edge0;
+  if (!edge0 && (save || rd != CLIPK_F32)) {
     if (rd == CLIPK_F32) {
       TRY(clipk_rows_copy(W * 4, rows, x0, nullptr, t.X[0], nullptr, st));
     } else {
@@ -731,6 +756,8 @@
   const bool fold = ln_fold_on(e, io);
   t_osplit = io.text ? o_split_on(e, sh, fold) : vit_o_split_on(e, sh, fold, save);
   if (save) e->o_saved_split = t_osplit;
+  const bool edgeL = text_edge_last(e, sh, io) && fold && (!save || t_osplit);
+  if (save) e->edgeL_saved = edgeL;
   bool have_stats = false;
   bool xs_ready = false;
   for (int l = 0; l < nl; ++l) {
@@ -742,12 +769,17 @@
     float* r1 = save ? t.rstd1[l] : t.tr;
     float* m2 = save ? t.mean2[l] : t.tm;
     float* r2 = save ? t.rstd2[l] : t.tr;
-    if (share0)
+    if (share0) {
       TRY(block_attn_shared0(e, e->lw[l], sh, rd, cur, t.xn, t.qkv[l], t.o[l], t.lse[l], t.mean1[l], t.rstd1[l],
                              (int*)t.g, st));
-    else if (fold && have_stats)
+      if (edge0) {
+        ProfScope ps(CLIPK_PROF_NONE, st, 0.0, "text.x0_prefix", 2.0 * sh.G * sh.P * W * 4);
+        TRY(clipk_rows_copy(W * 4, sh.G * sh.P, x0, (const int*)t.g, t.X[0], (const int*)t.g, st));
+      }
+    } else if (fold && have_stats)
       TRY(block_attn_fold(e, e->fold[l], sh, cur, t.qkv[l], t.o[l], t.lse[l], m1, r1, t.lnst, t.rnb, st, io.text,
-                          e->split == 2 ? (const float*)e->lw[l][0] : nullptr, xs_ready ? t.xn : nullptr));
+                          e->split == 2 ? (const float*)e->lw[l][0] : nullptr, xs_ready ? t.xn : nullptr,
+                          edgeL && l == nl - 1 ? CLIPK_PREFIX_EOT_QUERIES : 0));
     else
       TRY(block_attn(e, e->lw[l], sh, rd, cur, t.xn, t.qkv[l], t.o[l], t.lse[l], t.mean1[l], t.rstd1[l], st,
                      io.text, io.sk, io.skb));
@@ -804,6 +836,20 @@
   return CLIPK_OK;
 }
 
+__global__ __launch_bounds__(256) void zero_cols16_kernel(long n, int chunks, int stride, uint4* __restrict__ p) {
+  for (long i = (long)blockIdx.x * 256 + threadIdx.x; i < n; i += (long)gridDim.x * 256)
+    p[(i / chunks) * stride + i % chunks] = make_uint4(0, 0, 0, 0);
+}
+static int zero_cols(void* p, long rows, size_t col_bytes, size_t stride_bytes, hipStream_t st) {
+  if (rows <= 0 || col_bytes == 0) return CLIPK_OK;
+  if ((col_bytes | stride_bytes | (uintptr_t)p) & 15 || col_bytes > stride_bytes) return CLIPK_ESHAPE;
+  const long n = rows * (long)(col_bytes / 16);
+  hipLaunchKernelGGL(zero_cols16_kernel, dim3((unsigned)std::min<long>((n + 255) / 256, 4096)), dim3(256), 0, st, n,
+                     (int)(col_bytes / 16), (int)(stride_bytes / 16), (uint4*)p);
+  CLIPK_CHECK_LAUNCH();
+  return CLIPK_OK;
+}
+
 static int text_backward_impl(const clipk_encoder* e, const SeqShape& sh, const int* eot_rows,
                               const float* dtxt, const void* saved, size_t saved_bytes, float* dx0,
                               void* ws, size_t ws_bytes, hipStream_t st, const EncIO& io) {
@@ -814,6 +860,9 @@
   const int W = e->W, rows = sh.rows, nout = sh.nout, gd = e->grad, act = e->act;
   const int pg = io.text ? CLIPK_PROF_GEMM_ALL : CLIPK_PROF_NONE;
   if (e->o_saved_split && !prefix_split_bwd(e, sh, gd)) return CLIPK_EINVAL;
+  if (e->edge0_saved && !(io.text && prefix_mode(e, sh))) return CLIPK_EINVAL;
+  const bool edgeL = text_edge_last(e, sh, io);
+  if (e->edgeL_saved && !edgeL) return CLIPK_EINVAL;
   float* dX = dx0;
   if (e->split) {
     TRY(grad_scale_in(e, (long)nout * e->E, dtxt, (float*)b.dtg, b.gscale, st));
@@ -882,20 +931,25 @@
       void* res = r16 ? b.dX_lp : (void*)dX;
       ProfScope ps(CLIPK_PROF_NONE, st, 0.0, SITE("eot_scatter"),
                    2.0 * nout * (gb + 2.0 * rb) + (double)rows * (gb + rb));
-      TRY(zero(b.do_, (size_t)rows * gb));
+      if (!edgeL) TRY(zero(b.do_, (size_t)rows * gb));
       TRY(clipk_rows_copy(gb, nout, b.dh, nullptr, b.do_, eot_rows, st));
       TRY(clipk_rows_copy(rb, nout, res, nullptr, b.dqkv, nullptr, st));
       TRY(zero(res, (size_t)rows * rb));
       TRY(clipk_rows_copy(rb, nout, b.dqkv, nullptr, res, eot_rows, st));
+      if (edgeL) TRY(zero_cols(b.dqkv, rows, (size_t)W * 4, (size_t)3 * W * 4, st));
     }
     {
       const bool reads_o = act == CLIPK_F32 && !prefix_split_bwd(e, sh, gd);
-      const double ab = (double)rows * W * ((reads_o ? 4.0 : 3.0) * esize(act) + 4.0 * esize(gd)) +
-                        4.0 * rows * e->heads;
+      const bool eotq = compact && edgeL;
+      const double ab = eotq ? ((double)rows * 4 + (double)nout * 3) * W * 4.0 + 4.0 * nout * e->heads
+                             : (double)rows * W * ((reads_o ? 4.0 : 3.0) * esize(act) + 4.0 * esize(gd)) +
+                                   4.0 * rows * e->heads;
       ProfScope ps(io.text ? CLIPK_PROF_ATTN : CLIPK_PROF_NONE, st, 0.0, SITE("attn_bwd"), ab);
       const bool shared0 = l == 0 && io.text && sh.G >= 2 && prefix_mode(e, sh) && share0_index_on();
+      const bool edge0 = l == 0 && e->edge0_saved && prefix_split_bwd(e, sh, gd);
       TRY(attn_bwd(e, sh, t.qkv[l], t.o[l], b.do_, t.lse[l], b.dqkv, b.part, st, qkv_split,
-                   shared0 ? CLIPK_PREFIX_CLS_GROUP0 : 0));
+                   (shared0 ? CLIPK_PREFIX_CLS_GROUP0 : 0) | (edge0 ? CLIPK_PREFIX_GRAD_PREFIX : 0) |
+                       (eotq ? CLIPK_PREFIX_EOT_QUERIES : 0)));
     }
     if (lora_grad && ((lo.layer_mask >> l) & 1u)) {
       ProfScope ps(CLIPK_PROF_NONE, st, 0.0, SITE("lora_wgrad"), 2.0 * rows * W * (esize(rd) + 3.0 * esize(gd)));
diff --git a/include/clipk.h b/include/clipk.h
--- a/include/clipk.h
+++ b/include/clipk.h
@@ -139,7 +139,13 @@
                                const float* lse, void* dqkv, int lddqkv, void* ws, size_t ws_bytes,
                                void* stream);
 
-enum { CLIPK_PREFIX_CLS_GROUP0 = 1, CLIPK_PREFIX_SPLIT = 2, CLIPK_PREFIX_OUT_SPLIT = 4 };
+enum {
+  CLIPK_PREFIX_CLS_GROUP0 = 1,
+  CLIPK_PREFIX_SPLIT = 2,
+  CLIPK_PREFIX_OUT_SPLIT = 4,
+  CLIPK_PREFIX_GRAD_PREFIX = 8,
+  CLIPK_PREFIX_EOT_QUERIES = 16
+};
 int clipk_attention_prefix_fwd_ex(int dtype, int G, int P, int R, int ntiles, const int* tiles,
                                   const int* row_first, int heads, const void* qkv, int ldqkv, void* out,
                                   int ldo, float* lse, int flags, void* stream);
```

Result: no change. 385.1 (-0.3%).
